# simonsobs/pixell

Measured on AMD Instinct MI355X. Metric: map2alm+alm2map round-trips/sec, higher is better.
Workload: dtype f64

## Files before the change

pixell_amd/csrc/leg_s0.hip:

```cpp
#include "legendre_dev.hpp"

namespace pxs {

#define S0_PHASE_A \
	while (k + 4 <= nk) { \
		bool act = false; \
		_Pragma("unroll") for (int s = 0; s < K; s++) act |= LEG_IS_LIVE(lam2[s], sc[s]); \
		if (__any(act)) break; \
		const double4_t q0 = LDC(coef, k), q1 = LDC(coef, k+1), q2 = LDC(coef, k+2), q3 = LDC(coef, k+3); \
		const double b0 = polar ? q0.c : q0.b, b1 = polar ? q1.c : q1.b, b2 = polar ? q2.c : q2.b, b3 = polar ? q3.c : q3.b; \
		_Pragma("unroll") for (int s = 0; s < K; s++) { \
			lam1[s] = fma(fma(q0.a, csq[s], b0), lam2[s], lam1[s]); \
			lam2[s] = fma(fma(q1.a, csq[s], b1), lam1[s], lam2[s]); \
			lam1[s] = fma(fma(q2.a, csq[s], b2), lam2[s], lam1[s]); \
			lam2[s] = fma(fma(q3.a, csq[s], b3), lam1[s], lam2[s]); \
			if (sc[s] < 0 && fabs(lam2[s]) > SC_BIG) { lam1[s] *= SC_SMALL; lam2[s] *= SC_SMALL; sc[s]++; } \
		} \
		k += 4; \
	}
#define S0_SEEDED_PHASE_A \
	if (a.seed_mode == 2) { \
		const double* sd = a.seed_d + ((long)m*a.nwave + wv)*(2*K*64); const int* si = a.seed_i + ((long)m*a.nwave + wv)*((K+1)*64); \
		k = PXS_UNIFORM_INT(si[K*64]); \
		_Pragma("unroll") for (int s = 0; s < K; s++) { lam1[s] = sd[s*64 + lane]; lam2[s] = sd[(K+s)*64 + lane]; sc[s] = si[s*64 + lane]; } \
	} else { \
		S0_PHASE_A \
		if (a.seed_mode == 1) { \
			double* sd = a.seed_d + ((long)m*a.nwave + wv)*(2*K*64); int* si = a.seed_i + ((long)m*a.nwave + wv)*((K+1)*64); \
			_Pragma("unroll") for (int s = 0; s < K; s++) { sd[s*64 + lane] = lam1[s]; sd[(K+s)*64 + lane] = lam2[s]; si[s*64 + lane] = sc[s]; } \
			if (lane == 0) si[K*64] = k; \
		} \
	}

#define S0_SYN_PAIR(c0, c1, a0, a1) S0_SYN_PAIR_C(c0.a, polar ? c0.c : c0.b, c1.a, polar ? c1.c : c1.b, a0, a1)
#define S0_SYN_PAIR_C(ca0, cb0, ca1, cb1, a0, a1) { \
	PXS_VCOPY(vb0, cb0); \
	PXS_VCOPY(vb1, cb1); \
	_Pragma("unroll") for (int s = 0; s < K; s++) { \
		p1r[s] = fma(lam2[s], a0.a, p1r[s]); p1i[s] = fma(lam2[s], a0.b, p1i[s]); \
		p2r[s] = fma(lam2[s], a0.c, p2r[s]); p2i[s] = fma(lam2[s], a0.d, p2i[s]); \
		lam1[s] = fma(fma(ca0, csq[s], vb0), lam2[s], lam1[s]); \
	} \
	_Pragma("unroll") for (int s = 0; s < K; s++) { \
		p1r[s] = fma(lam1[s], a1.a, p1r[s]); p1i[s] = fma(lam1[s], a1.b, p1i[s]); \
		p2r[s] = fma(lam1[s], a1.c, p2r[s]); p2i[s] = fma(lam1[s], a1.d, p2i[s]); \
		lam2[s] = fma(fma(ca1, csq[s], vb1), lam1[s], lam2[s]); \
	} }

template<int K> __global__ __launch_bounds__(64, (K == 4 ? 7 : 1)) void leg_syn_s0(const LegK a)
{
	const int lane = threadIdx.x; int wv, m, bb;
	if (!leg_block(a, wv, m, bb)) return;
	const long row0 = PXS_UNIFORM_LONG(a.row[m]);
	const int nk = (a.lmax - m)/2 + 1;
	const double4_t* __restrict__ coef = a.coef + row0;
	const double4_t* __restrict__ at = reinterpret_cast<const double4_t*>(a.almt + (long)bb*a.almt_bs) + row0;
	double x[K], csq[K], lam1[K], lam2[K], p1r[K], p1i[K], p2r[K], p2i[K];
	int sc[K], rn[K], rs[K];
	bool alive_any = false;
	const bool polar = leg_wave_polar(a, wv, K);
#pragma unroll
	for (int s = 0; s < K; s++) {
		const int p = leg_pair_u(a, wv, K, s, lane);
		const bool valid = leg_pair_valid(a, p);
		rn[s] = valid ? a.ring_n[p] : -1; rs[s] = valid ? a.ring_s[p] : -1;
		x[s] = valid ? a.cth[p] : 0.0;
		const double sth = valid ? a.sth[p] : 0.0;
		csq[s] = polar ? -sth*sth : x[s]*x[s];
		const bool alive = valid && ((double)m <= a.lmax*sth + a.ofs);
		lam1[s] = 0; lam2[s] = 0; sc[s] = 0;
		if (alive && a.seed_mode != 2) { double mt; int e; pow_scaled(sth, m, mt, e); to_scaled(mt, e, lam2[s], sc[s]); }
		p1r[s] = p1i[s] = p2r[s] = p2i[s] = 0;
		alive_any |= alive;
	}
	int k = 0;
	if (__any(alive_any)) {
		S0_SEEDED_PHASE_A
		k = PXS_UNIFORM_INT(k); coef = (const double4_t*)PXS_UNIFORM_LONG((long)coef);
		PXS_COUNT(0, (long)(nk - k)*K*6 + (a.seed_mode != 2 ? (long)k*K*2 : 0L));
		while (k + 1 < nk) {
			bool pend = false;
#pragma unroll
			for (int s = 0; s < K; s++) pend |= (sc[s] < 0);
			if (!__any(pend)) break;
			for (int it = 0; it < 2 && k + 1 < nk; it++, k += 2) {
				const double4_t c0 = LDC(coef, k), c1 = LDC(coef, k+1), a0 = LDC(at, k), a1 = LDC(at, k+1);
				S0_SYN_PAIR(c0, c1, a0, a1)
			}
#pragma unroll
			for (int s = 0; s < K; s++)
				if (sc[s] < 0 && fabs(lam2[s]) > SC_BIG) {
					lam1[s] *= SC_SMALL; lam2[s] *= SC_SMALL;
					if (++sc[s] == 0) p1r[s] = p1i[s] = p2r[s] = p2i[s] = 0;
				}
		}
#pragma unroll
		for (int s = 0; s < K; s++) if (sc[s] < 0) { p1r[s] = p1i[s] = p2r[s] = p2i[s] = 0; lam1[s] = lam2[s] = 0; }
		const double2* __restrict__ cf = (const double2*)PXS_UNIFORM_LONG((long)((polar ? a.coef2p : a.coef2) + row0));
		coef2x2_t f = LDC2(cf, k); double4_t a0 = LDC(at, k), a1 = LDC(at, k+1);
		while (k + 3 < nk) {
			PXS_ROWS_DRAIN();
			coef2x2_t n = LDC2(cf, k+2); double4_t m0 = LDC(at, k+2), m1 = LDC(at, k+3);
			PXS_ROWS_ISSUED();
			S0_SYN_PAIR_C(f.a0, f.b0, f.a1, f.b1, a0, a1)
			PXS_ROWS_DRAIN();
			f = LDC2(cf, k+4); a0 = LDC(at, k+4); a1 = LDC(at, k+5);
			PXS_ROWS_ISSUED();
			S0_SYN_PAIR_C(n.a0, n.b0, n.a1, n.b1, m0, m1)
			k += 4;
		}
		for (; k + 1 < nk; k += 2) {
			PXS_ROWS_DRAIN();
			const coef2x2_t n = LDC2(cf, k+2); const double4_t m0 = LDC(at, k+2), m1 = LDC(at, k+3);
			PXS_ROWS_ISSUED();
			S0_SYN_PAIR_C(f.a0, f.b0, f.a1, f.b1, a0, a1)
			f = n; a0 = m0; a1 = m1;
		}
		PXS_ROWS_DRAIN();
		if (k < nk) {
#pragma unroll
			for (int s = 0; s < K; s++) {
				p1r[s] = fma(lam2[s], a0.a, p1r[s]); p1i[s] = fma(lam2[s], a0.b, p1i[s]);
				p2r[s] = fma(lam2[s], a0.c, p2r[s]); p2i[s] = fma(lam2[s], a0.d, p2i[s]);
			}
		}
	}
	double2* __restrict__ out = a.leg + (long)bb*a.leg_bs + (long)m*a.ld;
#pragma unroll
	for (int s = 0; s < K; s++) {
		const int p = leg_pair_u(a, wv, K, s, lane);
		const bool valid = leg_pair_valid(a, p);
		const int rn_ = valid ? a.ring_n[p] : -1, rs_ = valid ? a.ring_s[p] : -1;
		const double x_ = valid ? a.cth[p] : 0.0;
		if (rn_ >= 0) out[rn_] = make_double2(p1r[s] + x_*p2r[s], p1i[s] + x_*p2i[s]);
		if (rs_ >= 0) out[rs_] = make_double2(p1r[s] - x_*p2r[s], p1i[s] - x_*p2i[s]);
	}
}

#define S0_ANA_PAIR(c0, c1) { \
	PXS_VCOPY(vb0, polar ? c0.c : c0.b); \
	PXS_VCOPY(vb1, polar ? c1.c : c1.b); \
	double t0 = 0, t1 = 0, t2 = 0, t3 = 0, u0 = 0, u1 = 0, u2 = 0, u3 = 0; \
	_Pragma("unroll") for (int s = 0; s < K; s++) { \
		t0 = fma(lam2[s], d1r[s], t0); t1 = fma(lam2[s], d1i[s], t1); t2 = fma(lam2[s], d2r[s], t2); t3 = fma(lam2[s], d2i[s], t3); \
		lam1[s] = fma(fma(c0.a, csq[s], vb0), lam2[s], lam1[s]); \
	} \
	_Pragma("unroll") for (int s = 0; s < K; s++) { \
		u0 = fma(lam1[s], d1r[s], u0); u1 = fma(lam1[s], d1i[s], u1); u2 = fma(lam1[s], d2r[s], u2); u3 = fma(lam1[s], d2i[s], u3); \
		lam2[s] = fma(fma(c1.a, csq[s], vb1), lam1[s], lam2[s]); \
	} \
	 \
	LEG_RED_PUT(kk, t0, t1, t2, t3) \
	LEG_RED_PUT(kk+1, u0, u1, u2, u3) \
	kk += 2; \
	if (kk == LEG_FSTEPS) { leg_flush(red, pout + 4*kbase, lane, LEG_FSTEPS, a.atomic); kk = 0; kbase = k+2; } }

#define S0_ANA_STEP_C(ca, cb, LA, LB, T0, T1, T2, T3) { \
	PXS_VCOPY(vb, cb); \
	_Pragma("unroll") for (int s = 0; s < K; s++) { \
		T0 = fma(LA[s], d1r[s], T0); T1 = fma(LA[s], d1i[s], T1); T2 = fma(LA[s], d2r[s], T2); T3 = fma(LA[s], d2i[s], T3); \
		LB[s] = fma(fma(ca, csq[s], vb), LA[s], LB[s]); \
	} }
#define S0_ANA_PAIR_D(ca0, cb0, ca1, cb1, kfirst, NEXT) { \
	double t0 = 0, t1 = 0, t2 = 0, t3 = 0, u0 = 0, u1 = 0, u2 = 0, u3 = 0; \
	S0_ANA_STEP_C(ca0, cb0, lam2, lam1, t0, t1, t2, t3) \
	_Pragma("unroll") for (int s = 0; s < K; s++) PXS_DONE(lam1[s]); \
	PXS_DONE(t0); PXS_DONE(t1); PXS_DONE(t2); PXS_DONE(t3); \
	PXS_ROWS_DRAIN(); \
	if (kk == LEG_FSTEPS) { leg_flush(red, pout + 4*kbase, lane, LEG_FSTEPS, a.atomic); kk = 0; kbase = (kfirst); } \
	NEXT; \
	PXS_ROWS_ISSUED(); \
	S0_ANA_STEP_C(ca1, cb1, lam1, lam2, u0, u1, u2, u3) \
	LEG_RED_PUT(kk, t0, t1, t2, t3) \
	LEG_RED_PUT(kk+1, u0, u1, u2, u3) \
	kk += 2; }

template<int K> __global__ __launch_bounds__(64) void leg_ana_s0(const LegK a)
{
	PXS_SHARED(double, red);
	const int lane = threadIdx.x; int wv, m, bb;
	if (!leg_block(a, wv, m, bb)) return;
	const long row0 = PXS_UNIFORM_LONG(a.row[m]);
	const int nk = (a.lmax - m)/2 + 1;
	const double4_t* __restrict__ coef = a.coef + row0;
	double* __restrict__ pout = a.part + (long)bb*a.mom_bs + ((long)wv*a.rows_chunk + (row0 - a.rowbase))*4;
	const double2* __restrict__ in = a.leg + (long)bb*a.leg_bs + (long)m*a.ld;
	double csq[K], lam1[K], lam2[K], d1r[K], d1i[K], d2r[K], d2i[K];
	int sc[K];
	bool alive_any = false;
	const bool polar = leg_wave_polar(a, wv, K);
	auto load_data = [&](int s) {
		const int p = leg_pair(a, wv, K, s, PXS_LATE_INT(lane));
		const bool valid = leg_pair_valid(a, p);
		const int rn = valid ? a.ring_n[p] : -1, rs = valid ? a.ring_s[p] : -1;
		const double x = valid ? a.cth[p] : 0.0;
		const double2 vn = rn >= 0 ? in[rn] : make_double2(0, 0);
		const double2 vs = rs >= 0 ? in[rs] : make_double2(0, 0);
		d1r[s] = vn.x + vs.x; d1i[s] = vn.y + vs.y;
		d2r[s] = (vn.x - vs.x)*x; d2i[s] = (vn.y - vs.y)*x;
	};
#pragma unroll
	for (int s = 0; s < K; s++) {
		const int p = leg_pair(a, wv, K, s, lane);
		const bool valid = leg_pair_valid(a, p);
		const double x = valid ? a.cth[p] : 0.0;
		const double sth = valid ? a.sth[p] : 0.0;
		csq[s] = polar ? -sth*sth : x*x;
		const bool alive = valid && ((double)m <= a.lmax*sth + a.ofs);
		lam1[s] = 0; lam2[s] = 0; sc[s] = 0;
		if (alive && a.seed_mode != 2) { double mt; int e; pow_scaled(sth, m, mt, e); to_scaled(mt, e, lam2[s], sc[s]); }
		d1r[s] = d1i[s] = d2r[s] = d2i[s] = 0;
		alive_any |= alive;
	}
	if (!__any(alive_any)) return;
	int k = 0;
	S0_SEEDED_PHASE_A
	k = PXS_UNIFORM_INT(k); coef = (const double4_t*)PXS_UNIFORM_LONG((long)coef);
	PXS_COUNT(1, (long)(nk - k)*K*6 + (a.seed_mode != 2 ? (long)k*K*2 : 0L));
	if (lane == 0 && !a.atomic) a.first[wv*a.nmc + (m - a.m0)] = k + 1;
#pragma unroll
	for (int s = 0; s < K; s++) if (sc[s] == 0) load_data(s);
	int kk = 0, kbase = k;
	while (k + 1 < nk) {
		bool pend = false;
#pragma unroll
		for (int s = 0; s < K; s++) pend |= (sc[s] < 0);
		if (!__any(pend)) break;
		for (int it = 0; it < 2 && k + 1 < nk; it++, k += 2) {
			const double4_t c0 = LDC(coef, k), c1 = LDC(coef, k+1);
			S0_ANA_PAIR(c0, c1)
		}
#pragma unroll
		for (int s = 0; s < K; s++)
			if (sc[s] < 0 && fabs(lam2[s]) > SC_BIG) {
				lam1[s] *= SC_SMALL; lam2[s] *= SC_SMALL;
				if (++sc[s] == 0) load_data(s);
			}
	}
	const double2* __restrict__ cf = (const double2*)PXS_UNIFORM_LONG((long)((polar ? a.coef2p : a.coef2) + row0));
	coef2x2_t n = LDC2(cf, k), f = LDC2(cf, k+1);
	PXS_ROWS_DRAIN();
	n.a1 = n.a0; n.b1 = n.b0;
	while (k + 3 < nk) {
		S0_ANA_PAIR_D(n.a1, n.b1, f.a0, f.b0, k, n = LDC2(cf, k+3))
		S0_ANA_PAIR_D(f.a1, f.b1, n.a0, n.b0, k+2, f = LDC2(cf, k+5))
		k += 4;
	}
	if (k + 1 < nk) {
		S0_ANA_PAIR_D(n.a1, n.b1, f.a0, f.b0, k, (void)0)
		k += 2;
	}
	PXS_ROWS_DRAIN();
	if (kk == LEG_FSTEPS) { leg_flush(red, pout + 4*kbase, lane, LEG_FSTEPS, a.atomic); kk = 0; kbase = k; }
	if (k < nk) {
		double t0 = 0, t1 = 0, t2 = 0, t3 = 0;
#pragma unroll
		for (int s = 0; s < K; s++) { t0 = fma(lam2[s], d1r[s], t0); t1 = fma(lam2[s], d1i[s], t1); t2 = fma(lam2[s], d2r[s], t2); t3 = fma(lam2[s], d2i[s], t3); }
		LEG_RED_PUT(kk, t0, t1, t2, t3)
		kk++;
	}
	if (kk > 0) leg_flush(red, pout + 4*kbase, lane, kk, a.atomic);
}


struct S0Chain {
	double csq, lam1, lam2; int sc;
	__device__ __forceinline__ double step(double ca, double cb) { const double p = lam2, nx = fma(mm_coef(ca, csq, cb), lam2, lam1); lam1 = p; lam2 = nx; return p; }
	__device__ __forceinline__ void rescale() { if (fabs(lam2) > SC_BIG) { lam1 *= SC_SMALL; lam2 *= SC_SMALL; sc++; } }
	__device__ __forceinline__ void park_sign(int, double*) const {}
};
struct S0Mm {
	typedef S0Chain Chain;
	static constexpr int SLOTS = 64;
	static constexpr bool SIGNED = false;
	static constexpr bool BREG_SYNC = true;
	static __device__ __forceinline__ int steps(const LegK& a, int m, int& par) { par = 0; return (a.lmax - m)/2 + 1; }
	static __device__ __forceinline__ bool init(const LegK& a, int p, int m, int, bool polar, S0Chain& C) {
		const bool valid = p < a.npairs;
		const double x = valid ? a.cth[p] : 0.0, sth = valid ? a.sth[p] : 0.0;
		C.csq = polar ? -sth*sth : x*x;
		const bool alive = valid && ((double)m <= a.lmax*sth + a.ofs);
		C.lam1 = 0; C.lam2 = 0; C.sc = 0;
		if (alive) { double mt; int e; pow_scaled(sth, m, mt, e); to_scaled(mt, e, C.lam2, C.sc); }
		return alive;
	}
	static __device__ __forceinline__ const double* table(const LegK& a, bool polar, long row0) { return reinterpret_cast<const double*>(polar ? a.coef2p : a.coef2) + 2*row0; }
	static __device__ __forceinline__ int phase_a(const LegK& a, S0Chain& C, long row0, bool polar, int nk) {
		const double4_t* __restrict__ coef = a.coef + row0;
		int k = 0;
		while (k + 4 <= nk) {
			if (__any(LEG_IS_LIVE(C.lam2, C.sc))) break;
			const double4_t q0 = LDC(coef, k), q1 = LDC(coef, k+1), q2 = LDC(coef, k+2), q3 = LDC(coef, k+3);
			const double b0 = polar ? q0.c : q0.b, b1 = polar ? q1.c : q1.b, b2 = polar ? q2.c : q2.b, b3 = polar ? q3.c : q3.b;
			C.lam1 = fma(fma(q0.a, C.csq, b0), C.lam2, C.lam1);
			C.lam2 = fma(fma(q1.a, C.csq, b1), C.lam1, C.lam2);
			C.lam1 = fma(fma(q2.a, C.csq, b2), C.lam2, C.lam1);
			C.lam2 = fma(fma(q3.a, C.csq, b3), C.lam1, C.lam2);
			if (C.sc < 0) C.rescale();
			k += 4;
		}
		return k;
	}
	struct Data { double2 vn[4], vs[4]; };
	static __device__ __forceinline__ void load(const LegK& a, int m, int map0, int rn, int rs, Data& d) {
#pragma unroll
		for (int mm = 0; mm < 4; mm++) {
			const int map = map0 + mm;
			const double2* __restrict__ in = a.leg + (long)map*a.leg_bs + (long)m*a.ld;
			const bool okm = map < a.nmaps;
			d.vn[mm] = (okm && rn >= 0) ? in[rn] : make_double2(0, 0); d.vs[mm] = (okm && rs >= 0) ? in[rs] : make_double2(0, 0);
		}
	}
	static __device__ __forceinline__ void park(const Data& d, double x, int, double* __restrict__ ent) {
#pragma unroll
		for (int mm = 0; mm < 4; mm++) {
			ent[4*mm + 0] = d.vn[mm].x + d.vs[mm].x; ent[4*mm + 1] = d.vn[mm].y + d.vs[mm].y;
			ent[4*mm + 2] = (d.vn[mm].x - d.vs[mm].x)*x; ent[4*mm + 3] = (d.vn[mm].y - d.vs[mm].y)*x;
		}
	}
	template<int NG> static __device__ __forceinline__ void store(const LegK& a, int m, int bb, int pbase, int lane, mm_acc (&acc)[NG][4]) {
		const int c = lane & 3;
#pragma unroll
		for (int g = 0; g < NG; g++) {
			const int map = (bb*NG + g)*4 + ((lane & 15) >> 2);
			double* __restrict__ out = reinterpret_cast<double*>(a.leg + (long)(map < a.nmaps ? map : 0)*a.leg_bs + (long)m*a.ld) + (c & 1);
#pragma unroll
			for (int rb = 0; rb < 4; rb++)
#pragma unroll
				for (int r = 0; r < 4; r++) {
					const int p = pbase + 16*rb + 4*r + (lane >> 4);
					const bool valid = p < a.npairs && map < a.nmaps;
					const double v = acc[g][rb][r], o = MMS_XOR2(v);
					const double x = valid ? a.cth[p] : 0.0;
					const double val = c < 2 ? fma(x, o, v) : fma(-x, v, o);
					const int ring = valid ? (c < 2 ? a.ring_n[p] : a.ring_s[p]) : -1;
					if (ring >= 0) out[2*ring] = val;
				}
		}
	}
};
template<int NG, int W> __global__ __launch_bounds__(64*W, 4) void leg_ana_s0_mm(const LegK a) { leg_ana_mm<S0Mm, NG, W>(a); }



template<int NG> __global__ __launch_bounds__(64, 4) void leg_syn_s0_mm(const LegK a) { leg_syn_mm<S0Mm, NG>(a); }

void launch_leg_s0(bool analysis, int ng, int K, dim3 grid, hipStream_t st, const LegK& a) {
	static const bool once = leg_mm_lds_optin({leg_ana_s0_mm<2, MM_WAVES>, leg_ana_s0_mm<1, MM_WAVES>}); (void)once;
	const LegKernel k = analysis ? (ng == 2 ? leg_ana_s0_mm<2, MM_WAVES> : ng ? leg_ana_s0_mm<1, MM_WAVES> : K == 8 ? leg_ana_s0<8> : K == 4 ? leg_ana_s0<4> : K == 2 ? leg_ana_s0<2> : nullptr)
	                             : (ng == 2 ? leg_syn_s0_mm<2> : ng ? leg_syn_s0_mm<1> : K == 4 ? leg_syn_s0<4> : K == 2 ? leg_syn_s0<2> : nullptr);
	PXS_REQUIRE(k != nullptr, "internal: no spin-0 Legendre kernel compiled for this number of ring pairs per lane");
	leg_launch(k, analysis, ng, grid, st, a);
}

}
```

pixell_amd/csrc/leg_spin.hip:

```cpp
#include "legendre_dev.hpp"

namespace pxs {

template<int K> struct SpinState {
	double x[K], gp1[K], gp2[K], gm1[K], gm2[K];
	int scp[K], scm[K];
};

template<int K> __device__ __forceinline__ bool spin_init(const LegK& a, int wv, int lane, int m, SpinState<K>& S, int* rn, int* rs, bool polar) {
	const int s_ = a.spin;
	bool alive_any = false;
#pragma unroll
	for (int s = 0; s < K; s++) {
		const int p = leg_pair(a, wv, K, s, lane);
		const bool valid = leg_pair_valid(a, p);
		rn[s] = valid ? a.ring_n[p] : -1; rs[s] = valid ? a.ring_s[p] : -1;
		const double cth = valid ? a.cth[p] : 0.0;
		const double sth = valid ? a.sth[p] : 0.0;
		const double shh = valid ? a.sh2[p] : 0.0;
		S.x[s] = polar ? -2.0*shh*shh : cth;
		const double t1 = a.lmax*sth + a.ofs;
		const double b = -2.0*s_*fabs(cth);
		const double c = (double)s_*s_ - t1*t1;
		const double discr = b*b - 4*c;
		const double mlim = discr <= 0 ? a.lmax : fmin((double)a.lmax, 0.5*(-b + sqrt(discr)));
		const bool alive = valid && ((double)m <= mlim + 0.5);
		S.gp1[s] = S.gm1[s] = 0; S.gp2[s] = S.gm2[s] = 0; S.scp[s] = S.scm[s] = 0;
		if (alive && a.seed_mode != 2) {
			const double sh = shh, ch = a.ch2[p];
			double m1, m2; int e1, e2;
			if (m >= s_) {
				pow_scaled(sh, m + s_, m1, e1); pow_scaled(ch, m - s_, m2, e2);
				double mt = m1*m2; int e = e1 + e2 + m; frexp_norm(mt, e); to_scaled(mt, e, S.gp2[s], S.scp[s]);
				pow_scaled(sh, m - s_, m1, e1); pow_scaled(ch, m + s_, m2, e2);
				mt = m1*m2; e = e1 + e2 + m; frexp_norm(mt, e); to_scaled(mt, e, S.gm2[s], S.scm[s]);
			} else {
				pow_scaled(sh, s_ + m, m1, e1); pow_scaled(ch, s_ - m, m2, e2);
				double mt = m1*m2; int e = e1 + e2; frexp_norm(mt, e); to_scaled(mt, e, S.gp2[s], S.scp[s]);
				pow_scaled(sh, s_ - m, m1, e1); pow_scaled(ch, s_ + m, m2, e2);
				mt = m1*m2; e = e1 + e2; frexp_norm(mt, e); to_scaled(mt, e, S.gm2[s], S.scm[s]);
				if ((s_ - m) & 1) S.gm2[s] = -S.gm2[s];
			}
		}
		alive_any |= alive;
	}
	return alive_any;
}

#define SPIN_PHASE_A \
	while (j + 4 <= nl) { \
		bool act = false; \
		_Pragma("unroll") for (int s = 0; s < K; s++) act |= LEG_IS_LIVE(S.gp2[s], S.scp[s]) || LEG_IS_LIVE(S.gm2[s], S.scm[s]); \
		if (__any(act)) break; \
		const double4_t q0 = LDC(coef, j), q1 = LDC(coef, j+1), q2 = LDC(coef, j+2), q3 = LDC(coef, j+3); \
		_Pragma("unroll") for (int s = 0; s < K; s++) { \
			double ax; \
			ax = q0.a*S.x[s]; S.gp1[s] = fma(ax + (polar ? q0.c : q0.b), S.gp2[s], -S.gp1[s]); S.gm1[s] = fma(ax + (polar ? q0.d : -q0.b), S.gm2[s], -S.gm1[s]); \
			ax = q1.a*S.x[s]; S.gp2[s] = fma(ax + (polar ? q1.c : q1.b), S.gp1[s], -S.gp2[s]); S.gm2[s] = fma(ax + (polar ? q1.d : -q1.b), S.gm1[s], -S.gm2[s]); \
			ax = q2.a*S.x[s]; S.gp1[s] = fma(ax + (polar ? q2.c : q2.b), S.gp2[s], -S.gp1[s]); S.gm1[s] = fma(ax + (polar ? q2.d : -q2.b), S.gm2[s], -S.gm1[s]); \
			ax = q3.a*S.x[s]; S.gp2[s] = fma(ax + (polar ? q3.c : q3.b), S.gp1[s], -S.gp2[s]); S.gm2[s] = fma(ax + (polar ? q3.d : -q3.b), S.gm1[s], -S.gm2[s]); \
			if (S.scp[s] < 0 && fabs(S.gp2[s]) > SC_BIG) { S.gp1[s] *= SC_SMALL; S.gp2[s] *= SC_SMALL; S.scp[s]++; } \
			if (S.scm[s] < 0 && fabs(S.gm2[s]) > SC_BIG) { S.gm1[s] *= SC_SMALL; S.gm2[s] *= SC_SMALL; S.scm[s]++; } \
		} \
		j += 4; \
	}

#define SPIN_SEEDED_PHASE_A \
	if (a.seed_mode == 2) { \
		const double* sd = a.seed_d + ((long)m*a.nwave + wv)*(4*K*64); const int* si = a.seed_i + ((long)m*a.nwave + wv)*((2*K+1)*64); \
		j = PXS_UNIFORM_INT(si[2*K*64]); \
		_Pragma("unroll") for (int s = 0; s < K; s++) { \
			S.gp1[s] = sd[s*64 + lane]; S.gp2[s] = sd[(K+s)*64 + lane]; S.gm1[s] = sd[(2*K+s)*64 + lane]; S.gm2[s] = sd[(3*K+s)*64 + lane]; \
			S.scp[s] = si[s*64 + lane]; S.scm[s] = si[(K+s)*64 + lane]; } \
	} else { \
		SPIN_PHASE_A \
		if (a.seed_mode == 1) { \
			double* sd = a.seed_d + ((long)m*a.nwave + wv)*(4*K*64); int* si = a.seed_i + ((long)m*a.nwave + wv)*((2*K+1)*64); \
			_Pragma("unroll") for (int s = 0; s < K; s++) { \
				sd[s*64 + lane] = S.gp1[s]; sd[(K+s)*64 + lane] = S.gp2[s]; sd[(2*K+s)*64 + lane] = S.gm1[s]; sd[(3*K+s)*64 + lane] = S.gm2[s]; \
				si[s*64 + lane] = S.scp[s]; si[(K+s)*64 + lane] = S.scm[s]; } \
			if (lane == 0) si[2*K*64] = j; \
		} \
	}

struct spin_rows_t { double4_t r0, r1; };
__device__ __forceinline__ spin_rows_t spin_rows(const double4_t* coef, long i) { spin_rows_t r; r.r0 = LDC(coef, i); r.r1 = LDC(coef, i+1); return r; }
#define SPIN_ROW0(r) r.r0.a, polar ? r.r0.c : r.r0.b, polar ? r.r0.d : -r.r0.b
#define SPIN_ROW1(r) r.r1.a, polar ? r.r1.c : r.r1.b, polar ? r.r1.d : -r.r1.b

#define SPIN_SYN_PAIR(f0, f1, a0, a1) SPIN_SYN_PAIR_C(f0.a, polar ? f0.c : f0.b, polar ? f0.d : -f0.b, f1.a, polar ? f1.c : f1.b, polar ? f1.d : -f1.b, a0, a1)
#define SPIN_SYN_PAIR_C(ca0, c10, c20, ca1, c11, c21, a0, a1) { \
	{ \
		const double ca = ca0, c1 = c10, c2 = c20; \
		PXS_VCOPY(v1, c1); PXS_VCOPY(v2, c2); \
		_Pragma("unroll") for (int s = 0; s < K; s++) { \
			const double gp = S.gp2[s], gm = S.gm2[s]; \
			pnr[s] = fma(gp, a0.a, pnr[s]); pni[s] = fma(gp, a0.b, pni[s]); \
			mnr[s] = fma(gm, a0.c, mnr[s]); mni[s] = fma(gm, a0.d, mni[s]); \
			qsr[s] = fma(gm, a0.a, qsr[s]); qsi[s] = fma(gm, a0.b, qsi[s]); \
			nsr[s] = fma(gp, a0.c, nsr[s]); nsi[s] = fma(gp, a0.d, nsi[s]); \
			S.gp1[s] = fma(fma(ca, S.x[s], v1), gp, -S.gp1[s]); S.gm1[s] = fma(fma(ca, S.x[s], v2), gm, -S.gm1[s]); \
		} \
	} \
	{ \
		const double ca = ca1, c1 = c11, c2 = c21; \
		PXS_VCOPY(v1, c1); PXS_VCOPY(v2, c2); \
		_Pragma("unroll") for (int s = 0; s < K; s++) { \
			const double gp = S.gp1[s], gm = S.gm1[s]; \
			pnr[s] = fma(gp, a1.a, pnr[s]); pni[s] = fma(gp, a1.b, pni[s]); \
			mnr[s] = fma(gm, a1.c, mnr[s]); mni[s] = fma(gm, a1.d, mni[s]); \
			qsr[s] = fma(-gm, a1.a, qsr[s]); qsi[s] = fma(-gm, a1.b, qsi[s]); \
			nsr[s] = fma(-gp, a1.c, nsr[s]); nsi[s] = fma(-gp, a1.d, nsi[s]); \
			S.gp2[s] = fma(fma(ca, S.x[s], v1), gp, -S.gp2[s]); S.gm2[s] = fma(fma(ca, S.x[s], v2), gm, -S.gm2[s]); \
		} \
	} }

#define SPIN_SYN_PAIR_R(s0, s1, a0, a1) SPIN_SYN_PAIR_C(s0, s1, a0, a1)
#define SPIN_SYN_PHASE_C { \
	spin_rows_t f = spin_rows(coef, j); a0 = LDC(at, j); a1 = LDC(at, j+1); \
	while (j + 3 < nl) { \
		PXS_ROWS_DRAIN(); \
		spin_rows_t n = spin_rows(coef, j+2); double4_t m0 = LDC(at, j+2), m1 = LDC(at, j+3); \
		PXS_ROWS_ISSUED(); \
		SPIN_SYN_PAIR_R(SPIN_ROW0(f), SPIN_ROW1(f), a0, a1) \
		PXS_ROWS_DRAIN(); \
		f = spin_rows(coef, j+4); a0 = LDC(at, j+4); a1 = LDC(at, j+5); \
		PXS_ROWS_ISSUED(); \
		SPIN_SYN_PAIR_R(SPIN_ROW0(n), SPIN_ROW1(n), m0, m1) \
		j += 4; \
	} \
	for (; j + 1 < nl; j += 2) { \
		PXS_ROWS_DRAIN(); \
		const spin_rows_t n = spin_rows(coef, j+2); const double4_t m0 = LDC(at, j+2), m1 = LDC(at, j+3); \
		PXS_ROWS_ISSUED(); \
		SPIN_SYN_PAIR_R(SPIN_ROW0(f), SPIN_ROW1(f), a0, a1) \
		f = n; a0 = m0; a1 = m1; \
	} \
	PXS_ROWS_DRAIN(); }

template<int K> __global__ __launch_bounds__(64) void leg_syn_spin(const LegK a)
{
	const int lane = threadIdx.x; int wv, m, bb;
	if (!leg_block(a, wv, m, bb)) return;
	const int l0 = max(m, a.spin);
	const int nl = a.lmax - l0 + 1;
	double2* __restrict__ outq = a.leg + (long)bb*a.leg_bs + (long)m*a.ld;
	double2* __restrict__ outu = a.leg + (long)bb*a.leg_bs + ((long)a.nm + m)*a.ld;
	SpinState<K> S; int rn[K], rs[K];
	double pnr[K], pni[K], mnr[K], mni[K], qsr[K], qsi[K], nsr[K], nsi[K];
#pragma unroll
	for (int s = 0; s < K; s++) pnr[s] = pni[s] = mnr[s] = mni[s] = qsr[s] = qsi[s] = nsr[s] = nsi[s] = 0;
	const bool polar = leg_wave_polar(a, wv, K);
	const bool alive_any = spin_init<K>(a, wv, lane, m, S, rn, rs, polar);
	double sg0 = 1.0;
	if (nl > 0 && __any(alive_any)) {
		const long row0 = PXS_UNIFORM_LONG(a.row[m]);
		const double4_t* __restrict__ coef = a.coef + row0;
		const double4_t* __restrict__ at = reinterpret_cast<const double4_t*>(a.almt + (long)bb*a.almt_bs) + row0;
		int j = 0;
		SPIN_SEEDED_PHASE_A
		j = PXS_UNIFORM_INT(j); coef = (const double4_t*)PXS_UNIFORM_LONG((long)coef);
		PXS_COUNT(0, (long)(nl - j)*K*12 + (a.seed_mode != 2 ? (long)j*K*4 : 0L));
		sg0 = ((l0 + j + m) & 1) ? -1.0 : 1.0;
		while (j + 1 < nl) {
			bool pend = false;
#pragma unroll
			for (int s = 0; s < K; s++) pend |= (S.scp[s] < 0) || (S.scm[s] < 0);
			if (!__any(pend)) break;
			for (int it = 0; it < 2 && j + 1 < nl; it++, j += 2) {
				const double4_t f0 = LDC(coef, j), f1 = LDC(coef, j+1), a0 = LDC(at, j), a1 = LDC(at, j+1);
				SPIN_SYN_PAIR(f0, f1, a0, a1)
			}
#pragma unroll
			for (int s = 0; s < K; s++) {
				const bool was = (S.scp[s] < 0) || (S.scm[s] < 0);
				if (S.scp[s] < 0 && fabs(S.gp2[s]) > SC_BIG) { S.gp1[s] *= SC_SMALL; S.gp2[s] *= SC_SMALL; S.scp[s]++; }
				if (S.scm[s] < 0 && fabs(S.gm2[s]) > SC_BIG) { S.gm1[s] *= SC_SMALL; S.gm2[s] *= SC_SMALL; S.scm[s]++; }
				if (was && S.scp[s] == 0 && S.scm[s] == 0) pnr[s] = pni[s] = mnr[s] = mni[s] = qsr[s] = qsi[s] = nsr[s] = nsi[s] = 0;
			}
		}
#pragma unroll
		for (int s = 0; s < K; s++)
			if (S.scp[s] < 0 || S.scm[s] < 0) {
				pnr[s] = pni[s] = mnr[s] = mni[s] = qsr[s] = qsi[s] = nsr[s] = nsi[s] = 0;
				S.gp1[s] = S.gp2[s] = S.gm1[s] = S.gm2[s] = 0;
			}
		double4_t a0, a1;
		SPIN_SYN_PHASE_C
		if (j < nl) {
#pragma unroll
			for (int s = 0; s < K; s++) {
				const double gp = S.gp2[s], gm = S.gm2[s];
				pnr[s] = fma(gp, a0.a, pnr[s]); pni[s] = fma(gp, a0.b, pni[s]);
				mnr[s] = fma(gm, a0.c, mnr[s]); mni[s] = fma(gm, a0.d, mni[s]);
				qsr[s] = fma(gm, a0.a, qsr[s]); qsi[s] = fma(gm, a0.b, qsi[s]);
				nsr[s] = fma(gp, a0.c, nsr[s]); nsi[s] = fma(gp, a0.d, nsi[s]);
			}
		}
	}
#pragma unroll
	for (int s = 0; s < K; s++) {
		const int p = leg_pair(a, wv, K, s, lane);
		const bool valid = leg_pair_valid(a, p);
		const int rn_ = valid ? a.ring_n[p] : -1, rs_ = valid ? a.ring_s[p] : -1;
		if (rn_ >= 0) {
			outq[rn_] = make_double2(0.5*(pnr[s] + mnr[s]), 0.5*(pni[s] + mni[s]));
			outu[rn_] = make_double2(0.5*(pni[s] - mni[s]), -0.5*(pnr[s] - mnr[s]));
		}
		if (rs_ >= 0) {
			const double psr = sg0*qsr[s], psi = sg0*qsi[s], msr = sg0*nsr[s], msi = sg0*nsi[s];
			outq[rs_] = make_double2(0.5*(psr + msr), 0.5*(psi + msi));
			outu[rs_] = make_double2(0.5*(psi - msi), -0.5*(psr - msr));
		}
	}
}

#define SPIN_ANA_PAIR(f0, f1) { \
	double t0 = 0, t1 = 0, t2 = 0, t3 = 0, u0 = 0, u1 = 0, u2 = 0, u3 = 0; \
	{ \
		const double ca = f0.a, c1 = polar ? f0.c : f0.b, c2 = polar ? f0.d : -f0.b; \
		PXS_VCOPY(v1, c1); PXS_VCOPY(v2, c2); \
		_Pragma("unroll") for (int s = 0; s < K; s++) { \
			const double gp = S.gp2[s], gm = S.gm2[s]; \
			t0 = fma(gp, tpnr[s], t0); t0 = fma(gm, tpsr[s], t0); \
			t1 = fma(gp, tpni[s], t1); t1 = fma(gm, tpsi[s], t1); \
			t2 = fma(gm, tmnr[s], t2); t2 = fma(gp, tmsr[s], t2); \
			t3 = fma(gm, tmni[s], t3); t3 = fma(gp, tmsi[s], t3); \
			S.gp1[s] = fma(fma(ca, S.x[s], v1), gp, -S.gp1[s]); S.gm1[s] = fma(fma(ca, S.x[s], v2), gm, -S.gm1[s]); \
		} \
	} \
	{ \
		const double ca = f1.a, c1 = polar ? f1.c : f1.b, c2 = polar ? f1.d : -f1.b; \
		PXS_VCOPY(v1, c1); PXS_VCOPY(v2, c2); \
		_Pragma("unroll") for (int s = 0; s < K; s++) { \
			const double gp = S.gp1[s], gm = S.gm1[s]; \
			u0 = fma(gp, tpnr[s], u0); u0 = fma(-gm, tpsr[s], u0); \
			u1 = fma(gp, tpni[s], u1); u1 = fma(-gm, tpsi[s], u1); \
			u2 = fma(gm, tmnr[s], u2); u2 = fma(-gp, tmsr[s], u2); \
			u3 = fma(gm, tmni[s], u3); u3 = fma(-gp, tmsi[s], u3); \
			S.gp2[s] = fma(fma(ca, S.x[s], v1), gp, -S.gp2[s]); S.gm2[s] = fma(fma(ca, S.x[s], v2), gm, -S.gm2[s]); \
		} \
	} \
	 \
	LEG_RED_PUT(kk, t0, t1, t2, t3) \
	LEG_RED_PUT(kk+1, u0, u1, u2, u3) \
	kk += 2; \
	if (kk == LEG_FSTEPS) { leg_flush(red, pout + 4*jbase, lane, LEG_FSTEPS, a.atomic); kk = 0; jbase = j+2; } }

#define SPIN_ANA_STEP0_C(ca, c1, c2) { \
	PXS_VCOPY(v1, c1); PXS_VCOPY(v2, c2); \
	_Pragma("unroll") for (int s = 0; s < K; s++) { \
		const double gp = S.gp2[s], gm = S.gm2[s]; \
		t0 = fma(gp, tpnr[s], t0); t0 = fma(gm, tpsr[s], t0); \
		t1 = fma(gp, tpni[s], t1); t1 = fma(gm, tpsi[s], t1); \
		t2 = fma(gm, tmnr[s], t2); t2 = fma(gp, tmsr[s], t2); \
		t3 = fma(gm, tmni[s], t3); t3 = fma(gp, tmsi[s], t3); \
		S.gp1[s] = fma(fma(ca, S.x[s], v1), gp, -S.gp1[s]); S.gm1[s] = fma(fma(ca, S.x[s], v2), gm, -S.gm1[s]); \
	} }
#define SPIN_ANA_STEP1_C(ca, c1, c2) { \
	PXS_VCOPY(v1, c1); PXS_VCOPY(v2, c2); \
	_Pragma("unroll") for (int s = 0; s < K; s++) { \
		const double gp = S.gp1[s], gm = S.gm1[s]; \
		u0 = fma(gp, tpnr[s], u0); u0 = fma(-gm, tpsr[s], u0); \
		u1 = fma(gp, tpni[s], u1); u1 = fma(-gm, tpsi[s], u1); \
		u2 = fma(gm, tmnr[s], u2); u2 = fma(-gp, tmsr[s], u2); \
		u3 = fma(gm, tmni[s], u3); u3 = fma(-gp, tmsi[s], u3); \
		S.gp2[s] = fma(fma(ca, S.x[s], v1), gp, -S.gp2[s]); S.gm2[s] = fma(fma(ca, S.x[s], v2), gm, -S.gm2[s]); \
	} }
#define SPIN_ANA_PAIR_D(ca0, c10, c20, ca1, c11, c21, jfirst, NEXT) { \
	double t0 = 0, t1 = 0, t2 = 0, t3 = 0, u0 = 0, u1 = 0, u2 = 0, u3 = 0; \
	SPIN_ANA_STEP0_C(ca0, c10, c20) \
	_Pragma("unroll") for (int s = 0; s < K; s++) { PXS_DONE(S.gp1[s]); PXS_DONE(S.gm1[s]); } \
	PXS_DONE(t0); PXS_DONE(t1); PXS_DONE(t2); PXS_DONE(t3); \
	PXS_ROWS_DRAIN(); \
	if (kk == LEG_FSTEPS) { leg_flush(red, pout + 4*jbase, lane, LEG_FSTEPS, a.atomic); kk = 0; jbase = (jfirst); } \
	NEXT; \
	PXS_ROWS_ISSUED(); \
	SPIN_ANA_STEP1_C(ca1, c11, c21) \
	LEG_RED_PUT(kk, t0, t1, t2, t3) \
	LEG_RED_PUT(kk+1, u0, u1, u2, u3) \
	kk += 2; }
#define SPIN_ANA_PHASE_C { \
	spin_rows_t n = spin_rows(coef, j), f = spin_rows(coef, j+1); \
	PXS_ROWS_DRAIN(); \
	n.r1 = n.r0; \
	while (j + 3 < nl) {       \
		SPIN_ANA_PAIR_R(SPIN_ROW1(n), SPIN_ROW0(f), j, n = spin_rows(coef, j+3)) \
		SPIN_ANA_PAIR_R(SPIN_ROW1(f), SPIN_ROW0(n), j+2, f = spin_rows(coef, j+5)) \
		j += 4; \
	} \
	if (j + 1 < nl) { \
		SPIN_ANA_PAIR_R(SPIN_ROW1(n), SPIN_ROW0(f), j, (void)0) \
		j += 2; \
	} }
#define SPIN_ANA_PAIR_R(s0, s1, jfirst, NEXT) SPIN_ANA_PAIR_D(s0, s1, jfirst, NEXT)

template<int K> __global__ __launch_bounds__(64, (K == 2 ? 5 : 1)) void leg_ana_spin(const LegK a)
{
	PXS_SHARED(double, red);
	const int lane = threadIdx.x; int wv, m, bb;
	if (!leg_block(a, wv, m, bb)) return;
	const int l0 = max(m, a.spin);
	const int nl = a.lmax - l0 + 1;
	if (nl <= 0) return;
	const long row0 = PXS_UNIFORM_LONG(a.row[m]);
	const double4_t* __restrict__ coef = a.coef + row0;
	double* __restrict__ pout = a.part + (long)bb*a.mom_bs + ((long)wv*a.rows_chunk + (row0 - a.rowbase))*4;
	const double2* __restrict__ inq = a.leg + (long)bb*a.leg_bs + (long)m*a.ld;
	const double2* __restrict__ inu = a.leg + (long)bb*a.leg_bs + ((long)a.nm + m)*a.ld;
	SpinState<K> S; int rn[K], rs[K];
	const bool polar = leg_wave_polar(a, wv, K);
	const bool alive_any = spin_init<K>(a, wv, lane, m, S, rn, rs, polar);
	if (!__any(alive_any)) return;
	const double sgn0 = ((l0 + m) & 1) ? -1.0 : 1.0;
	double tpnr[K], tpni[K], tmnr[K], tmni[K], tpsr[K], tpsi[K], tmsr[K], tmsi[K];
	auto load_data = [&](int s) {
		const int p = leg_pair(a, wv, K, s, PXS_LATE_INT(lane));
		const bool valid = leg_pair_valid(a, p);
		const int rn_ = valid ? a.ring_n[p] : -1, rs_ = valid ? a.ring_s[p] : -1;
		double2 q = rn_ >= 0 ? inq[rn_] : make_double2(0, 0), u = rn_ >= 0 ? inu[rn_] : make_double2(0, 0);
		tpnr[s] = q.x - u.y; tpni[s] = q.y + u.x; tmnr[s] = q.x + u.y; tmni[s] = q.y - u.x;
		q = rs_ >= 0 ? inq[rs_] : make_double2(0, 0); u = rs_ >= 0 ? inu[rs_] : make_double2(0, 0);
		tpsr[s] = sgn0*(q.x - u.y); tpsi[s] = sgn0*(q.y + u.x); tmsr[s] = sgn0*(q.x + u.y); tmsi[s] = sgn0*(q.y - u.x);
	};
#pragma unroll
	for (int s = 0; s < K; s++) tpnr[s] = tpni[s] = tmnr[s] = tmni[s] = tpsr[s] = tpsi[s] = tmsr[s] = tmsi[s] = 0;
	int j = 0;
	SPIN_SEEDED_PHASE_A
	j = PXS_UNIFORM_INT(j); coef = (const double4_t*)PXS_UNIFORM_LONG((long)coef);
	PXS_COUNT(1, (long)(nl - j)*K*12 + (a.seed_mode != 2 ? (long)j*K*4 : 0L));
	if (lane == 0 && !a.atomic) a.first[wv*a.nmc + (m - a.m0)] = j + 1;
#pragma unroll
	for (int s = 0; s < K; s++) if (S.scp[s] == 0 && S.scm[s] == 0) load_data(s);
	int kk = 0, jbase = j;
	while (j + 1 < nl) {
		bool pend = false;
#pragma unroll
		for (int s = 0; s < K; s++) pend |= (S.scp[s] < 0) || (S.scm[s] < 0);
		if (!__any(pend)) break;
		for (int it = 0; it < 2 && j + 1 < nl; it++, j += 2) {
			const double4_t f0 = LDC(coef, j), f1 = LDC(coef, j+1);
			SPIN_ANA_PAIR(f0, f1)
		}
#pragma unroll
		for (int s = 0; s < K; s++) {
			const bool was = (S.scp[s] < 0) || (S.scm[s] < 0);
			if (S.scp[s] < 0 && fabs(S.gp2[s]) > SC_BIG) { S.gp1[s] *= SC_SMALL; S.gp2[s] *= SC_SMALL; S.scp[s]++; }
			if (S.scm[s] < 0 && fabs(S.gm2[s]) > SC_BIG) { S.gm1[s] *= SC_SMALL; S.gm2[s] *= SC_SMALL; S.scm[s]++; }
			if (was && S.scp[s] == 0 && S.scm[s] == 0) load_data(s);
		}
	}
	SPIN_ANA_PHASE_C
	PXS_ROWS_DRAIN();
	if (kk == LEG_FSTEPS) { leg_flush(red, pout + 4*jbase, lane, LEG_FSTEPS, a.atomic); kk = 0; jbase = j; }
	if (j < nl) {
		double t0 = 0, t1 = 0, t2 = 0, t3 = 0;
#pragma unroll
		for (int s = 0; s < K; s++) {
			const double gp = S.gp2[s], gm = S.gm2[s];
			t0 = fma(gp, tpnr[s], t0); t0 = fma(gm, tpsr[s], t0);
			t1 = fma(gp, tpni[s], t1); t1 = fma(gm, tpsi[s], t1);
			t2 = fma(gm, tmnr[s], t2); t2 = fma(gp, tmsr[s], t2);
			t3 = fma(gm, tmni[s], t3); t3 = fma(gp, tmsi[s], t3);
		}
		LEG_RED_PUT(kk, t0, t1, t2, t3)
		kk++;
	}
	if (kk > 0) leg_flush(red, pout + 4*jbase, lane, kk, a.atomic);
}


struct SpinChain {
	double x, g1, g2, sgl, pa; int sc, half, par;
	__device__ __forceinline__ double coef(double ca, double cb) const { return fma(ca, x, fma(sgl, cb, pa*ca)); }
	__device__ __forceinline__ double step(double ca, double cb) { const double p = g2, nx = fma(coef(ca, cb), g2, -g1); g1 = p; g2 = nx; return p; }
	__device__ __forceinline__ void rescale() { if (fabs(g2) > SC_BIG) { g1 *= SC_SMALL; g2 *= SC_SMALL; sc++; } }
	__device__ __forceinline__ void park_sign(int kq, double* p) const {
		const double se = (half && ((par + kq) & 1)) ? -1.0 : 1.0, so = half ? -se : 1.0;
		p[0] *= se; p[1] *= so; p[2] *= se; p[3] *= so;
	}
};
struct SpinMm {
	typedef SpinChain Chain;
	static constexpr int SLOTS = 32;
	static constexpr bool SIGNED = true;
	static constexpr bool BREG_SYNC = false;
	static __device__ __forceinline__ int steps(const LegK& a, int m, int& par) { const int l0 = max(m, a.spin); par = l0 + m; return a.lmax - l0 + 1; }
	static __device__ __forceinline__ bool init(const LegK& a, int p, int m, int half, bool polar, SpinChain& C) {
		const int s_ = a.spin;
		const bool valid = p < a.npairs;
		const double cth = valid ? a.cth[p] : 0.0, sth = valid ? a.sth[p] : 0.0, shh = valid ? a.sh2[p] : 0.0;
		C.x = polar ? -2.0*shh*shh : cth; C.sgl = half ? -1.0 : 1.0; C.pa = polar ? 1.0 : 0.0; C.half = half; C.par = max(m, s_) + m;
		const double t1 = a.lmax*sth + a.ofs, b = -2.0*s_*fabs(cth), c = (double)s_*s_ - t1*t1, discr = b*b - 4*c;
		const double mlim = discr <= 0 ? a.lmax : fmin((double)a.lmax, 0.5*(-b + sqrt(discr)));
		const bool alive = valid && ((double)m <= mlim + 0.5);
		C.g1 = 0; C.g2 = 0; C.sc = 0;
		if (alive) {
			const double sh = shh, ch = a.ch2[p];
			double m1, m2; int e1, e2;
			const int es = m >= s_ ? (half ? m - s_ : m + s_) : (half ? s_ - m : s_ + m), ec = m >= s_ ? (half ? m + s_ : m - s_) : (half ? s_ + m : s_ - m);
			pow_scaled(sh, es, m1, e1); pow_scaled(ch, ec, m2, e2);
			double mt = m1*m2; int e = e1 + e2 + (m >= s_ ? m : 0); frexp_norm(mt, e); to_scaled(mt, e, C.g2, C.sc);
			if (m < s_ && half && ((s_ - m) & 1)) C.g2 = -C.g2;
		}
		return alive;
	}
	static __device__ __forceinline__ const double* table(const LegK& a, bool, long row0) { return reinterpret_cast<const double*>(a.coef2) + 2*row0; }
	static __device__ __forceinline__ int phase_a(const LegK& a, SpinChain& C, long row0, bool polar, int n) {
		const double* __restrict__ tab = table(a, polar, row0);
		int k = 0;
		while (k + 4 <= n) {
			if (__any(LEG_IS_LIVE(C.g2, C.sc))) break;
			double cq[8];
#pragma unroll
			for (int i = 0; i < 8; i++) cq[i] = LDCD(tab, 2L*k + i);
#pragma unroll
			for (int i = 0; i < 4; i++) C.step(cq[2*i], cq[2*i + 1]);
			if (C.sc < 0) C.rescale();
			k += 4;
		}
		return k;
	}
	struct Data { double2 qn[4], un[4], qs[4], us[4]; };
	static __device__ __forceinline__ void load(const LegK& a, int m, int map0, int rn, int rs, Data& d) {
#pragma unroll
		for (int mm = 0; mm < 4; mm++) {
			const int map = map0 + mm;
			const double2* __restrict__ inq = a.leg + (long)map*a.leg_bs + (long)m*a.ld;
			const double2* __restrict__ inu = a.leg + (long)map*a.leg_bs + ((long)a.nm + m)*a.ld;
			const bool okm = map < a.nmaps;
			d.qn[mm] = (okm && rn >= 0) ? inq[rn] : make_double2(0, 0); d.un[mm] = (okm && rn >= 0) ? inu[rn] : make_double2(0, 0);
			d.qs[mm] = (okm && rs >= 0) ? inq[rs] : make_double2(0, 0); d.us[mm] = (okm && rs >= 0) ? inu[rs] : make_double2(0, 0);
		}
	}
	static __device__ __forceinline__ void park(const Data& d, double, int half, double* __restrict__ ent) {
#pragma unroll
		for (int mm = 0; mm < 4; mm++) {
			const double tpn_r = d.qn[mm].x - d.un[mm].y, tpn_i = d.qn[mm].y + d.un[mm].x, tmn_r = d.qn[mm].x + d.un[mm].y, tmn_i = d.qn[mm].y - d.un[mm].x;
			const double tps_r = d.qs[mm].x - d.us[mm].y, tps_i = d.qs[mm].y + d.us[mm].x, tms_r = d.qs[mm].x + d.us[mm].y, tms_i = d.qs[mm].y - d.us[mm].x;
			ent[4*mm + 0] = half ? tps_r : tpn_r; ent[4*mm + 1] = half ? tps_i : tpn_i;
			ent[4*mm + 2] = half ? tmn_r : tms_r; ent[4*mm + 3] = half ? tmn_i : tms_i;
		}
	}
	template<int NG> static __device__ __forceinline__ void store(const LegK& a, int m, int bb, int pbase, int lane, mm_acc (&acc)[NG][4]) {
		const int c = lane & 3;
#pragma unroll
		for (int g = 0; g < NG; g++) {
			const int map = (bb*NG + g)*4 + ((lane & 15) >> 2);
			double* __restrict__ outq = reinterpret_cast<double*>(a.leg + (long)(map < a.nmaps ? map : 0)*a.leg_bs + (long)m*a.ld);
			double* __restrict__ outu = reinterpret_cast<double*>(a.leg + (long)(map < a.nmaps ? map : 0)*a.leg_bs + ((long)a.nm + m)*a.ld);
#pragma unroll
			for (int rb = 0; rb < 2; rb++)
#pragma unroll
				for (int r = 0; r < 4; r++) {
					const int p = pbase + 16*rb + 4*r + (lane >> 4);
					const bool valid = p < a.npairs && map < a.nmaps;
					const double own = acc[g][rb][r], oth = MMS_XOR2(acc[g][rb + 2][r]);
					const double P = c < 2 ? own : oth, M = c < 2 ? oth : own;
					const double sum = 0.5*(P + M), dif = 0.5*(P - M);
					const int ring = valid ? (c < 2 ? a.ring_n[p] : a.ring_s[p]) : -1;
					if (ring >= 0) {
						if (c & 1) { outq[2*ring + 1] = sum; outu[2*ring] = dif; }
						else       { outq[2*ring] = sum; outu[2*ring + 1] = -dif; }
					}
				}
		}
	}
};
template<int NG, int W> __global__ __launch_bounds__(64*W, 4) void leg_ana_spin_mm(const LegK a) { leg_ana_mm<SpinMm, NG, W>(a); }

template<int NG> __global__ __launch_bounds__(64, 4) void leg_syn_spin_mm(const LegK a) { leg_syn_mm<SpinMm, NG>(a); }

void launch_leg_spin(bool analysis, int ng, int K, dim3 grid, hipStream_t st, const LegK& a) {
	static const bool once = leg_mm_lds_optin({leg_ana_spin_mm<2, MM_WAVES>, leg_ana_spin_mm<1, MM_WAVES>}); (void)once;
	const LegKernel k = analysis ? (ng == 2 ? leg_ana_spin_mm<2, MM_WAVES> : ng ? leg_ana_spin_mm<1, MM_WAVES> : K == 6 ? leg_ana_spin<6> : K == 4 ? leg_ana_spin<4> : K == 3 ? leg_ana_spin<3> : K == 2 ? leg_ana_spin<2> : nullptr)
	                             : (ng == 2 ? leg_syn_spin_mm<2> : ng ? leg_syn_spin_mm<1> : K == 3 ? leg_syn_spin<3> : K == 2 ? leg_syn_spin<2> : nullptr);
	PXS_REQUIRE(k != nullptr, "internal: no spin-s Legendre kernel compiled for this number of ring pairs per lane");
	leg_launch(k, analysis, ng, grid, st, a);
}

}
```

pixell_amd/csrc/legendre_dev.hpp:

```cpp
#pragma once
#include "legendre.hpp"
#include <cmath>
#include <algorithm>
#include <initializer_list>

namespace pxs {

static constexpr double SC_BIG   = 0x1p+400;
static constexpr double SC_SMALL = 0x1p-800;
static constexpr int    SC_STEP  = 800;
static constexpr double LEG_LIVE = 0x1p-140;
#define LEG_IS_LIVE(v, sc) ((sc) == 0 && fabs(v) >= LEG_LIVE)

struct double4_t { double a, b, c, d; };
#ifdef PXS_HOST_SIM
#define LDC(p, i) ((p)[i])
#else
typedef double pxs_d4 __attribute__((ext_vector_type(4)));
__device__ __forceinline__ double4_t ldc_row(const double4_t* p, long i) {
	const __attribute__((address_space(4))) pxs_d4* c = (const __attribute__((address_space(4))) pxs_d4*)(unsigned long long)p;
	const pxs_d4 v = c[i]; double4_t r; r.a = v.x; r.b = v.y; r.c = v.z; r.d = v.w; return r;
}
#define LDC(p, i) ldc_row((p), (i))
#endif
#ifdef PXS_HOST_SIM
#define LDCD(p, i) ((p)[i])
#else
__device__ __forceinline__ double ldc_double(const double* p, long i) {
	const __attribute__((address_space(4))) double* c = (const __attribute__((address_space(4))) double*)(unsigned long long)p;
	return c[i];
}
#define LDCD(p, i) ldc_double((p), (i))
#endif

struct coef2x2_t { double a0, b0, a1, b1; };
#ifdef PXS_HOST_SIM
#define LDC2(p, i) (coef2x2_t{(p)[i].x, (p)[i].y, (p)[(i)+1].x, (p)[(i)+1].y})
#define PXS_ROWS_DRAIN()
#define PXS_ROWS_ISSUED()
#else
typedef double pxs_d4a16 __attribute__((ext_vector_type(4), aligned(16)));
__device__ __forceinline__ coef2x2_t ldc_row2(const double2* p, long i) {
	const __attribute__((address_space(4))) pxs_d4a16* c = (const __attribute__((address_space(4))) pxs_d4a16*)(unsigned long long)(p + i);
	const pxs_d4a16 v = *c; coef2x2_t r; r.a0 = v.x; r.b0 = v.y; r.a1 = v.z; r.b1 = v.w; return r;
}
#define LDC2(p, i) ldc_row2((p), (i))
#define PXS_ROWS_DRAIN() do { __builtin_amdgcn_s_waitcnt(0xc07f); __builtin_amdgcn_sched_barrier(0); } while (0)
#define PXS_ROWS_ISSUED() __builtin_amdgcn_sched_barrier(0)
#endif
#ifdef PXS_HOST_SIM
#define PXS_DONE(x)
#else
#define PXS_DONE(x) asm volatile("" : "+v"(x))
#endif

struct LegK {
	int lmax, mmax, spin, nm, npairs, nring, nwave;
	long ld;
	long nrows;
	const long* row; const double4_t* coef; const double* alpha;
	const int* ring_n; const int* ring_s; const double* cth; const double* sth; const double* sh2; const double* ch2;
	double* almt; double* part; double* mom;
	double2* leg;
	double ofs;
	int m0; long rowbase, rows_chunk;
	int nmc, xcd;
	int* first;
	int atomic;
	int seed_mode; double* seed_d; int* seed_i;
	double* count;
	int nb; long leg_bs, almt_bs, mom_bs;
	int nmaps;
	const double2* coef2; const double2* coef2p;
};
#define PXS_NCOUNT 1024
#ifdef PXS_HOST_SIM
#define PXS_COUNT(dir, expr) if (a.count != nullptr && lane == 0) atomicAdd(a.count + 2*(blockIdx.x & (PXS_NCOUNT - 1)) + (dir), (double)(expr))
#else
#define PXS_COUNT(dir, expr) if (a.count != nullptr && lane == 0) unsafeAtomicAdd(a.count + 2*(blockIdx.x & (PXS_NCOUNT - 1)) + (dir), (double)(expr))
#endif

__host__ __device__ constexpr unsigned leg_blocks_per_m(unsigned nwave, unsigned nb) { return (nwave*nb) | 1u; }
static_assert(leg_blocks_per_m(20, 1) == 21 && leg_blocks_per_m(27, 1) == 27 && leg_blocks_per_m(4, 8) == 33 && leg_blocks_per_m(3, 2) == 7, "blocks per m: odd, at most one more than chunks x maps");
__device__ __forceinline__ bool leg_block(const LegK& a, int& wv, int& m, int& bb) {
	if (!a.xcd) { wv = blockIdx.x; m = blockIdx.y + a.m0; bb = blockIdx.z; return true; }
	const unsigned b = blockIdx.x, x = b & 7u, j = b >> 3;
	const unsigned per_m = leg_blocks_per_m((unsigned)a.nwave, (unsigned)a.nb);
	const unsigned ml = j / per_m, r = j - ml*per_m;
	bb = (int)(r / (unsigned)a.nwave);
	wv = (int)(r - (unsigned)bb*a.nwave);
	const unsigned mi = ml*8u + x;
	m = (int)mi + a.m0;
	return mi < (unsigned)a.nmc && bb < a.nb;
}
static inline dim3 leg_grid(const LegK& a) { return a.xcd ? dim3((unsigned)(8*((a.nmc+7)/8)*leg_blocks_per_m(a.nwave, a.nb))) : dim3(a.nwave, a.nmc, a.nb); }

__device__ __forceinline__ void frexp_norm(double& m, int& e) { int d; m = frexp(m, &d); e += d; }

__device__ __forceinline__ void pow_scaled(double x, int n, double& mant, int& e) {
	double rm = 0.5; int re = 1;
	int be = 0; double bm = frexp(x, &be);
	while (n) {
		if (n & 1) { rm *= bm; re += be; frexp_norm(rm, re); }
		bm *= bm; be *= 2; frexp_norm(bm, be);
		n >>= 1;
	}
	mant = rm; e = re;
}
__device__ __forceinline__ void to_scaled(double mant, int e, double& v, int& scale) {
	if (mant == 0.0) { v = 0.0; scale = 0; return; }
	int s = (e >= 0) ? (e + SC_STEP/2)/SC_STEP : -((-e + SC_STEP/2)/SC_STEP);
	if (s > 0) s = 0;
	v = ldexp(mant, e - SC_STEP*s); scale = s;
}

#ifndef PXS_POLAR_COS2
#define PXS_POLAR_COS2 0.1
#endif
__device__ __forceinline__ bool mm_wave_polar(const LegK& a, int end) {
	const double c = a.cth[min(end, a.npairs) - 1];
	return c*c > PXS_POLAR_COS2;
}
__host__ __device__ constexpr int leg_pair_of(int npairs, int nwave, int K, int wv, int s, int lane) { return (wv*K + s)*64 + lane - (nwave*K*64 - npairs); }
__host__ __device__ constexpr int leg_wave_last_pair(int npairs, int K, int wv) { return leg_pair_of(npairs, (npairs + 64*K - 1)/(64*K), K, wv, K - 1, 63); }
static_assert(leg_wave_last_pair(1451, 3, 0) == 106 && leg_wave_last_pair(1451, 4, 0) == 170 && leg_wave_last_pair(1451, 8, 0) == 426, "pair map: first wave");
static_assert(leg_wave_last_pair(1451, 3, 7) == 1450 && leg_wave_last_pair(1451, 4, 5) == 1450 && leg_wave_last_pair(1451, 8, 2) == 1450, "pair map: last wave");
static_assert(leg_pair_of(1451, 8, 3, 0, 0, 0) == -85 && leg_pair_of(1451, 8, 3, 0, 1, 21) == 0 && leg_pair_of(512, 2, 4, 0, 0, 0) == 0 && leg_wave_last_pair(30, 4, 0) == 29, "pair map: padding");
__device__ __forceinline__ int leg_pair(const LegK& a, int wv, int K, int s, int lane) { return leg_pair_of(a.npairs, a.nwave, K, wv, s, lane); }
__device__ __forceinline__ bool leg_pair_valid(const LegK& a, int p) { return (unsigned)p < (unsigned)a.npairs; }
__device__ __forceinline__ bool leg_wave_polar(const LegK& a, int wv, int K) { return mm_wave_polar(a, leg_wave_last_pair(a.npairs, K, wv) + 1); }

#ifdef PXS_HOST_SIM
#define PXS_VCOPY(dst, src) double dst = (src)
#else
#define PXS_VCOPY(dst, src) double dst; asm("v_mov_b64 %0, %1" : "=v"(dst) : "s"(src))
#endif

#ifdef PXS_HOST_SIM
#define PXS_FRESH_INT(x) (x)
#else
__device__ __forceinline__ int pxs_fresh_int(int x) { asm("" : "+v"(x)); return x; }
#define PXS_FRESH_INT(x) pxs_fresh_int(x)
#endif
#ifdef PXS_HOST_SIM
#define PXS_LATE_INT(x) (x)
#else
__device__ __forceinline__ int pxs_late_int(int x) { asm volatile("" : "+v"(x)); return x; }
#define PXS_LATE_INT(x) pxs_late_int(x)
#endif


#ifdef PXS_HOST_SIM
#define PXS_UNIFORM_INT(x) (x)
#define PXS_UNIFORM_LONG(x) (x)
#else
#define PXS_UNIFORM_INT(x) __builtin_amdgcn_readfirstlane(x)
#define PXS_UNIFORM_LONG(x) ((long)(((unsigned long)(unsigned)__builtin_amdgcn_readfirstlane((int)((unsigned long)(x) >> 32)) << 32) | (unsigned long)(unsigned)__builtin_amdgcn_readfirstlane((int)(unsigned long)(x))))
#endif
__device__ __forceinline__ int leg_pair_u(const LegK& a, int wv, int K, int s, int lane) { return PXS_UNIFORM_INT(leg_pair(a, wv, K, s, 0)) + lane; }


#ifdef PXS_HOST_SIM
#define PXS_WAVE_LDS_SYNC() pxsim::wave_sync()
#else
#define PXS_WAVE_LDS_SYNC() asm volatile("s_waitcnt lgkmcnt(0)" ::: "memory")
#endif
#define LEG_FSTEPS 16
#ifdef PXS_HOST_SIM
#define LEG_RED_STRIDE 66
#define LEG_RED_DOUBLES (4*LEG_FSTEPS*LEG_RED_STRIDE)
__device__ __forceinline__ double leg_flush_sum(const double* red, int lane) {
	const double* r = red + lane*LEG_RED_STRIDE;
	double s0 = 0, s1 = 0, s2 = 0, s3 = 0;
	for (int i = 0; i < 64; i += 4) { s0 += r[i]; s1 += r[i+1]; s2 += r[i+2]; s3 += r[i+3]; }
	return (s0 + s1) + (s2 + s3);
}
__device__ __forceinline__ int leg_flush_col(int lane) { return lane; }
#define LEG_RED_PUT(kk, t0, t1, t2, t3) \
	red[((kk)*4+0)*LEG_RED_STRIDE + lane] = t0; red[((kk)*4+1)*LEG_RED_STRIDE + lane] = t1; \
	red[((kk)*4+2)*LEG_RED_STRIDE + lane] = t2; red[((kk)*4+3)*LEG_RED_STRIDE + lane] = t3;
#else
#define LEG_RED_STRIDE 18
#define LEG_RED_DOUBLES (4*LEG_FSTEPS*LEG_RED_STRIDE)
__device__ __forceinline__ void leg_swap32(double& a, double& b) {
	const unsigned alo = __double2loint(a), ahi = __double2hiint(a), blo = __double2loint(b), bhi = __double2hiint(b);
	const auto r0 = __builtin_amdgcn_permlane32_swap(alo, blo, false, false);
	const auto r1 = __builtin_amdgcn_permlane32_swap(ahi, bhi, false, false);
	a = __hiloint2double(r1[0], r0[0]); b = __hiloint2double(r1[1], r0[1]);
}
__device__ __forceinline__ void leg_swap16(double& a, double& b) {
	const unsigned alo = __double2loint(a), ahi = __double2hiint(a), blo = __double2loint(b), bhi = __double2hiint(b);
	const auto r0 = __builtin_amdgcn_permlane16_swap(alo, blo, false, false);
	const auto r1 = __builtin_amdgcn_permlane16_swap(ahi, bhi, false, false);
	a = __hiloint2double(r1[0], r0[0]); b = __hiloint2double(r1[1], r0[1]);
}
__device__ __forceinline__ double leg_flush_sum(const double* red, int lane) {
	const double2* r = reinterpret_cast<const double2*>(red + lane*LEG_RED_STRIDE);
	double sum = 0;
#pragma unroll 1
	for (int h = 0; h < 8; h += 4) {
		const double2 a = r[h], b = r[h+1], c = r[h+2], d = r[h+3];
		sum += ((a.x + a.y) + (b.x + b.y)) + ((c.x + c.y) + (d.x + d.y));
	}
	return sum;
}
__device__ __forceinline__ int leg_flush_col(int lane) { const int r = lane & 3; return (lane & ~3) | ((r == 1) ? 2 : (r == 2) ? 1 : r); }
#define LEG_RED_PUT(kk, t0, t1, t2, t3) { \
	double a_ = t0, b_ = t1, c_ = t2, d_ = t3; \
	leg_swap32(a_, b_); leg_swap32(c_, d_); \
	double u_ = a_ + b_, v_ = c_ + d_; \
	leg_swap16(u_, v_); \
	red[((kk)*4 + (lane >> 4))*LEG_RED_STRIDE + (lane & 15)] = u_ + v_; }
#endif
__device__ __forceinline__ void leg_flush(double* red, double* __restrict__ dst, int lane, int nkk, int atomic) {
	PXS_WAVE_LDS_SYNC();
	if (lane < 4*nkk) {
		const double sum = leg_flush_sum(red, lane);
		double* q = dst + leg_flush_col(lane);
#ifdef PXS_HOST_SIM
		if (atomic) atomicAdd(q, sum); else *q = sum;
#else
		if (atomic) unsafeAtomicAdd(q, sum); else *q = sum;
#endif
	}
	PXS_WAVE_LDS_SYNC();
}


#define MM_PSTRIDE 65
#define MM_WAVES 8
#define MM_ESTRIDE 17
#ifdef PXS_HOST_SIM
struct mm_acc { double v[4]; double& operator[](int i) { return v[i]; } };
static inline mm_acc mm_mfma(double av, double bv, mm_acc c) {
	pxsim::BlockCtx* cx = pxsim::t_ctx; const int w = pxsim::wave_id(), l = pxsim::lane_id();
	uint64_t* s = cx->wslot->data() + (size_t)w*128;
	memcpy(&s[l], &av, 8); memcpy(&s[64 + l], &bv, 8); cx->wbar[w]->wait();
	for (int r = 0; r < 4; r++) {
		const int i = 4*r + (l >> 4), j = l & 15;
		double sum = c.v[r];
		for (int kk = 0; kk < 4; kk++) { double x, y; memcpy(&x, &s[i + 16*kk], 8); memcpy(&y, &s[64 + j + 16*kk], 8); sum = fma(x, y, sum); }
		c.v[r] = sum;
	}
	cx->wbar[w]->wait();
	return c;
}
static inline void mm_lds_add(double* p, double v) { atomicAdd(p, v); }
#define MM_WAVE_SYNC() pxsim::t_ctx->wbar[pxsim::wave_id()]->wait()
#else
typedef double mm_acc __attribute__((ext_vector_type(4)));
__device__ __forceinline__ mm_acc mm_mfma(double av, double bv, mm_acc c) { return __builtin_amdgcn_mfma_f64_16x16x4f64(av, bv, c, 0, 0, 0); }
__device__ __forceinline__ void mm_lds_add(double* p, double v) { (void)__hip_atomic_fetch_add(p, v, __ATOMIC_RELAXED, __HIP_MEMORY_SCOPE_WORKGROUP); }
#define MM_WAVE_SYNC() asm volatile("s_waitcnt lgkmcnt(0)" ::: "memory")
#endif
__device__ __forceinline__ double mm_coef(double ca, double x2, double cb) { PXS_VCOPY(vb_, cb); return fma(ca, x2, vb_); }
__device__ __forceinline__ void mm_load_cf(double (&cf)[32], const double* __restrict__ tab, int k0) {
#pragma unroll
	for (int i = 0; i < 32; i++) cf[i] = LDCD(tab, 2L*k0 + i);
}
template<int STRIDE, class Chain>
__device__ __forceinline__ void mm_park_tile(Chain& C, const double (&cf)[32], int k0, int kw, int n, bool& pend, double* __restrict__ ptile, int lane) {
#pragma unroll
	for (int q4 = 0; q4 < 4; q4++) {
		const int kq = k0 + 4*q4;
		double p[4] = {0, 0, 0, 0};
		if (kq >= kw && kq < n) {
#pragma unroll
			for (int i = 0; i < 4; i++) p[i] = C.step(cf[8*q4 + 2*i], cf[8*q4 + 2*i + 1]);
			if (pend) {
				if (C.sc < 0) { p[0] = p[1] = p[2] = p[3] = 0.0; C.rescale(); }
				pend = __any(C.sc < 0);
			}
			C.park_sign(kq, p);
			if (kq + 1 >= n) p[1] = 0.0;
			if (kq + 2 >= n) p[2] = 0.0;
			if (kq + 3 >= n) p[3] = 0.0;
		}
#pragma unroll
		for (int i = 0; i < 4; i++) ptile[(4*q4 + i)*STRIDE + lane] = p[i];
	}
}
template<int NG, bool SIGNED> struct MmSynB {
	const double* src[NG]; bool ok[NG]; int kk4, cc, par;
	__device__ __forceinline__ void init(const LegK& a, int bb, long row0, int lane, int par_) {
		const int jcol = lane & 15; kk4 = lane >> 4; cc = jcol & 3; par = par_;
#pragma unroll
		for (int g = 0; g < NG; g++) {
			const int map = (bb*NG + g)*4 + (jcol >> 2);
			ok[g] = map < a.nmaps;
			src[g] = a.almt + (long)(ok[g] ? map : 0)*a.almt_bs + 4*row0 + cc + 16*kk4;
		}
	}
	__device__ __forceinline__ void load(int k0, int n, double (*b)[4]) const {
#pragma unroll
		for (int g = 0; g < NG; g++)
#pragma unroll
			for (int q = 0; q < 4; q++) {
				const int row = k0 + q + 4*kk4;
				const double v = (ok[g] && row < n) ? src[g][4L*(k0 + q)] : 0.0;
				b[g][q] = (SIGNED && cc >= 2 && ((par + row) & 1)) ? -v : v;
			}
	}
};
template<int NG, int W, bool SIGNED>
__device__ __forceinline__ void mm_flush(const LegK& a, double* __restrict__ red, int tf, int w, int lane, int bb, int n, long row0, int par) {
	double* __restrict__ redf = red + (tf & 1)*NG*4*64;
	for (int cidx = w; cidx < 4*NG; cidx += W) {
		const int g = cidx >> 2, r = cidx & 3;
		double* rp = redf + cidx*64 + lane;
		double v = *rp; *rp = 0.0;
		const int krow = 16*tf + 4*r + (lane >> 4), map = (bb*NG + g)*4 + ((lane & 15) >> 2), c = lane & 3;
		if (krow < n && map < a.nmaps) {
			if (SIGNED && c >= 2 && ((par + krow) & 1)) v = -v;
			double* dst = a.mom + (long)map*a.mom_bs + 4*(row0 + krow) + c;
#ifdef PXS_HOST_SIM
			atomicAdd(dst, v);
#else
			unsafeAtomicAdd(dst, v);
#endif
		}
	}
}
__host__ __device__ constexpr int mm_lds_doubles(int NG, int W) { return W*16*MM_PSTRIDE + 2*NG*4*64 > 64*W*MM_ESTRIDE ? W*16*MM_PSTRIDE + 2*NG*4*64 : 64*W*MM_ESTRIDE; }
static inline size_t mm_ana_lds(int NG, int W) { return sizeof(double)*(size_t)mm_lds_doubles(NG, W) + 16; }

#define MMS_PSTRIDE 68
static inline size_t mm_syn_lds() { return sizeof(double)*16*MMS_PSTRIDE; }
#ifdef PXS_HOST_SIM
#define MMS_XOR2(v) __shfl_xor((v), 2)
#else
__device__ __forceinline__ double mms_xor2(double v) {
	const int lo = __builtin_amdgcn_mov_dpp(__double2loint(v), 0x4e, 0xf, 0xf, true), hi = __builtin_amdgcn_mov_dpp(__double2hiint(v), 0x4e, 0xf, 0xf, true);
	return __hiloint2double(hi, lo);
}
#define MMS_XOR2(v) mms_xor2(v)
#endif

template<class Sys, int NG, int W> __device__ __forceinline__ void leg_ana_mm(const LegK& a)
{
	PXS_SHARED(double, sh);
	double* __restrict__ ptile = sh;
	double* __restrict__ red = sh + W*16*MM_PSTRIDE;
	int* __restrict__ s_kmin = reinterpret_cast<int*>(sh + mm_lds_doubles(NG, W));
	const int tid = threadIdx.x, lane = tid & 63, w = PXS_UNIFORM_INT(tid >> 6), half = lane/Sys::SLOTS;
	int wv, m, bb;
	if (!leg_block(a, wv, m, bb)) return;
	int par;
	const int n = Sys::steps(a, m, par);
	if (n <= 0) return;
	const long row0 = PXS_UNIFORM_LONG(a.row[m]);
	const int pbase = wv*Sys::SLOTS*W;
	const bool polar = mm_wave_polar(a, pbase + Sys::SLOTS*(w + 1));
	const int pmine_ = pbase + Sys::SLOTS*w + (lane & (Sys::SLOTS - 1));
	typename Sys::Chain C;
	const bool alive = Sys::init(a, pmine_, m, half, polar, C);
	if (tid == 0) *s_kmin = n;
	__syncthreads();
	const bool wave_alive = __any(alive);
	const int kw = PXS_UNIFORM_INT(wave_alive ? Sys::phase_a(a, C, row0, polar, n) : n + 16);
	if (lane == 0) atomicMin(s_kmin, kw);
	__syncthreads();
	const int kmin = PXS_UNIFORM_INT(*s_kmin);
	if (kmin >= n) return;
	double breg[NG][16];
	{
		const bool ok = pmine_ < a.npairs;
		const int rn = ok ? a.ring_n[pmine_] : -1, rs = ok ? a.ring_s[pmine_] : -1;
		const double x = ok ? a.cth[pmine_] : 0.0;
		double* __restrict__ ent = sh + tid*MM_ESTRIDE;
		const double* __restrict__ rd = sh + (64*w + 16*(lane >> 4))*MM_ESTRIDE + (lane & 15);
#pragma unroll
		for (int g = 0; g < NG; g++) {
			typename Sys::Data d;
			Sys::load(a, m, (bb*NG + g)*4, rn, rs, d);
			if (g > 0) __syncthreads();
			Sys::park(d, x, half, ent);
			__syncthreads();
#pragma unroll
			for (int q = 0; q < 16; q++) breg[g][q] = rd[q*MM_ESTRIDE];
			if (Sys::BREG_SYNC) MM_WAVE_SYNC();
		}
		__syncthreads();
		for (int i = tid; i < 2*NG*4*64; i += 64*W) red[i] = 0.0;
		__syncthreads();
	}
	const double* __restrict__ tab = Sys::table(a, polar, row0);
	bool pend = __any(C.sc < 0);
	double* __restrict__ pmine = ptile + w*16*MM_PSTRIDE;
	const double* __restrict__ pread = pmine + (lane & 15)*MM_PSTRIDE + 16*(lane >> 4);
	double cf[32]; int cf_tile = -1;
	long ntile = 0;
	auto flush = [&](int tf) { mm_flush<NG, W, Sys::SIGNED>(a, red, tf, w, lane, bb, n, row0, par); };
	int tlast = -1;
	for (int t = kmin >> 4; 16*t < n; t++) {
		const int k0 = 16*t;
		double* __restrict__ redt = red + (t & 1)*NG*4*64;
		if (k0 + 16 > kw) {
			ntile++;
			if (cf_tile != t) mm_load_cf(cf, tab, k0);
			mm_park_tile<MM_PSTRIDE>(C, cf, k0, kw, n, pend, pmine, lane);
			MM_WAVE_SYNC();
			double av[4];
#pragma unroll
			for (int q = 0; q < 4; q++) av[q] = pread[q];
			MM_WAVE_SYNC();
			if (k0 + 16 < n) { mm_load_cf(cf, tab, k0 + 16); cf_tile = t + 1; }
			mm_acc acc[NG];
#pragma unroll
			for (int g = 0; g < NG; g++) { acc[g][0] = 0; acc[g][1] = 0; acc[g][2] = 0; acc[g][3] = 0; }
#pragma unroll
			for (int q = 0; q < 16; q++) {
				const double aq = q < 4 ? av[q] : pread[q];
#pragma unroll
				for (int g = 0; g < NG; g++) acc[g] = mm_mfma(aq, breg[g][q], acc[g]);
			}
			if (tlast >= 0) { flush(tlast); tlast = -1; }
#pragma unroll
			for (int g = 0; g < NG; g++)
#pragma unroll
				for (int r = 0; r < 4; r++) mm_lds_add(redt + (g*4 + r)*64 + lane, acc[g][r]);
		}
		if (tlast >= 0) flush(tlast);
		tlast = t;
		__syncthreads();
	}
	if (tlast >= 0) flush(tlast);
	PXS_COUNT(1, ntile*(NG*256L + 32L) + (wave_alive ? (long)kw*2 : 0L));
}

template<class Sys, int NG> __device__ __forceinline__ void leg_syn_mm(const LegK& a)
{
	PXS_SHARED(double, pmine);
	const int lane = threadIdx.x, half = lane/Sys::SLOTS;
	int wv, m, bb;
	if (!leg_block(a, wv, m, bb)) return;
	int par;
	const int n = Sys::steps(a, m, par);
	const long row0 = PXS_UNIFORM_LONG(a.row[m]);
	const int pbase = wv*Sys::SLOTS;
	const bool polar = mm_wave_polar(a, pbase + Sys::SLOTS);
	typename Sys::Chain C;
	const bool alive = Sys::init(a, pbase + (lane & (Sys::SLOTS - 1)), m, half, polar, C);
	mm_acc acc[NG][4];
#pragma unroll
	for (int g = 0; g < NG; g++)
#pragma unroll
		for (int rb = 0; rb < 4; rb++) { acc[g][rb][0] = 0; acc[g][rb][1] = 0; acc[g][rb][2] = 0; acc[g][rb][3] = 0; }
	long ntile = 0;
	const bool wave_alive = n > 0 && __any(alive);
	const int kw = PXS_UNIFORM_INT(wave_alive ? Sys::phase_a(a, C, row0, polar, n) : max(n, 0) + 16);
	{
		const double* __restrict__ tab = Sys::table(a, polar, row0);
		MmSynB<NG, Sys::SIGNED> B; B.init(a, bb, row0, lane, par);
		bool pend = __any(C.sc < 0);
		const double* __restrict__ pread = pmine + 4*(lane >> 4)*MMS_PSTRIDE + (lane & 15);
		double cf[32];
		double bcur[NG][4], bnxt[NG][4];
		B.load(16*(kw >> 4), n, bcur);
		if (kw < n) mm_load_cf(cf, tab, 16*(kw >> 4));
		for (int t = kw >> 4; 16*t < n; t++) {
			const int k0 = 16*t;
			ntile++;
			mm_park_tile<MMS_PSTRIDE>(C, cf, k0, kw, n, pend, pmine, lane);
			MM_WAVE_SYNC();
			double av[4];
#pragma unroll
			for (int rb = 0; rb < 4; rb++) av[rb] = pread[16*rb];
			MM_WAVE_SYNC();
			if (k0 + 16 < n) { mm_load_cf(cf, tab, k0 + 16); B.load(k0 + 16, n, bnxt); }
#pragma unroll
			for (int q = 0; q < 4; q++)
#pragma unroll
				for (int rb = 0; rb < 4; rb++) {
					const double aq = q == 0 ? av[rb] : pread[q*MMS_PSTRIDE + 16*rb];
#pragma unroll
					for (int g = 0; g < NG; g++) acc[g][rb] = mm_mfma(aq, bcur[g][q], acc[g][rb]);
				}
			MM_WAVE_SYNC();
#pragma unroll
			for (int g = 0; g < NG; g++)
#pragma unroll
				for (int q = 0; q < 4; q++) bcur[g][q] = bnxt[g][q];
		}
	}
	Sys::template store<NG>(a, m, bb, pbase, PXS_FRESH_INT(lane), acc);
	PXS_COUNT(0, ntile*(NG*256L + 32L) + (wave_alive ? (long)kw*2 : 0L));
}

typedef void (*LegKernel)(const LegK);
static inline bool leg_mm_lds_optin(std::initializer_list<LegKernel> ks) {
	for (LegKernel k : ks) (void)hipFuncSetAttribute((const void*)k, hipFuncAttributeMaxDynamicSharedMemorySize, 160*1024 - 256);
	return true;
}
static inline void leg_launch(LegKernel k, bool analysis, int ng, dim3 grid, hipStream_t st, const LegK& a) {
	const int W = analysis && ng ? MM_WAVES : 1;
	const size_t lds = ng ? (analysis ? mm_ana_lds(ng, MM_WAVES) : mm_syn_lds()) : analysis ? sizeof(double)*LEG_RED_DOUBLES : 0;
	hipLaunchKernelGGL(k, grid, dim3(64*W), lds, st, a);
}
void launch_leg_s0(bool analysis, int ng, int K, dim3 grid, hipStream_t st, const LegK& a);
void launch_leg_spin(bool analysis, int ng, int K, dim3 grid, hipStream_t st, const LegK& a);

}
```

pixell_amd/csrc/sht.hip:

```cpp
#include "sht_plan.hpp"
#include <cmath>
#include <algorithm>

static const char* const ROUTE_NAMES[] = {"direct", "via-cc", "via-cc-unfused", "via-cc-unfused-h", "ring-weights", "cc-weights", "chain", "unfused"};

Route::Scratch Route::scratch(const pxs_plan* p, int nb) const {
	Scratch s; const size_t nct = (size_t)nb*nc, nm = (size_t)p->mmax + 1, c16 = sizeof(double2);
	s.leg = c16*nct*nm*ld_leg_alloc; s.leg2 = c16*nct*nm*ld_leg2; s.h = c16*nct*nr_h*ld_h;
	if (to_map) s.almt = sizeof(double)*4*(tb->nrows + 4)*nb; else s.mom = sizeof(double)*4*std::max<long>(tb->nrows, 1)*nb;
	if (theta_fused && !line) FftChain::theta_scratch(theta, form->tp, (int)nm, (int)nct, s.c1, s.c2);
	if (reserve_chain) p->chain->ring_scratch(p->nring, (int)nct, !to_map, s.r1, p->mmax);
	return s;
}

namespace {

void plan_common(pxs_plan* p, int lmax, int mmax, const uint64_t* mstart, int64_t lstride, int device) {
	PXS_REQUIRE(lmax >= 0 && mmax >= 0 && mmax <= lmax, "need 0 <= mmax <= lmax");
	PXS_REQUIRE(mstart != nullptr, "mstart is required");
	PXS_HIP(hipSetDevice(device));
	p->device = device; p->lmax = lmax; p->mmax = mmax; p->lstride = lstride;
	std::vector<uint64_t> ms(mstart, mstart+mmax+1);
	p->d_mstart = upload(ms);
	p->fc = &fft_context(device);
	{
		size_t fr = 0, tot = 0;
		if (hipMemGetInfo(&fr, &tot) == hipSuccess && fr > 0) p->wk.part_budget = std::min<size_t>(size_t(2) << 30, std::max<size_t>(fr/8, size_t(256) << 20));
		env_budget("PXS_PART_GB", 30, p->wk.part_budget);
		{ const char* d = getenv("PXS_DETERMINISTIC"); p->wk.deterministic = d && atoi(d) != 0; }
	}
	env_budget("PXS_RESAMPLE_MB", 20, p->resample_chunk_bytes);
	{ const char* e = getenv("PXS_ANALYSIS"); if (e) { const std::string v(e); p->ana_weights = v == "weights" ? 1 : (v == "ducc0" ? 2 : (v == "interpolant" ? 0 : p->ana_weights)); } }
	if (p->general) return;
	std::string why;
	if (!FftContext::supported(p->nphi, &why)) throw Error(PXS_ERR_UNSUPPORTED, why);
	std::vector<double2> ph(mmax+1);
	for (int m = 0; m <= mmax; m++) { LDb a = (LDb)m*(LDb)p->phi0; ph[m] = make_double2((double)cosl(a), (double)(-sinl(a))); }
	p->phase = upload(ph);
	p->chain.reset(new FftChain(p->fc));
	p->chain_rings = 2L*mmax < p->nphi && p->chain->plan_rings(p->nphi);
	if (getenv("PXS_CHAIN_VERBOSE")) fprintf(stderr, "[pxsht] ring chain nphi=%d mmax=%d: %s\n", p->nphi, mmax, p->chain_rings ? p->chain->describe().c_str() : "off");
}

void setup_resampling(pxs_plan* p) {
	ThetaTables& t = p->th; AnaForm &ai = p->ana_interp, &af = p->ana_fine;
	af.fine = true;
	if (p->nfull == 0) p->nfull = p->nring;
	GridInfo gi = grid_info(p->geometry, p->nfull);
	t.N = gi.N; t.mir_c = gi.c;
	const int lmax = p->lmax;
	t.Ncc = FftContext::good_size(std::max<long>(2L*lmax + 2, 4));
	if (t.Ncc & 1) t.Ncc = FftContext::good_size(t.Ncc + 1);
	while (t.Ncc & 1) t.Ncc = FftContext::good_size(t.Ncc + 1);
	{
		const long nd = FftChain::ducc_ncc(lmax);
		if (nd >= 4 && FftContext::supported(nd) && FftContext::supported(2*nd)) t.Ncc = nd;
	}
	ai.M = FftContext::good_size(t.N + 2L*lmax + 2);
	if (p->chain_rings) {
		ai.tp = FftChain::plan_theta(t.N, lmax);
		if (ai.tp.ok) { t.Ncc = ai.tp.Ncc; ai.M = ai.tp.M; }
		if (getenv("PXS_CHAIN_VERBOSE")) fprintf(stderr, "[pxsht] theta chain N=%ld lmax=%d: ok=%d g=%ld bN=%ld g2=%ld (M=%ld) ac=%ld (Ncc=%ld) | syn gs=%ld bs=%ld aNs=%ld\n",
			t.N, lmax, (int)ai.tp.ok, ai.tp.g, ai.tp.bN, ai.tp.g2, ai.tp.M, ai.tp.ac, ai.tp.Ncc, ai.tp.gs, ai.tp.bs, ai.tp.aNs);
	}
	t.ncc = (int)(t.Ncc/2 + 1);
	std::string why;
	if (!FftContext::supported(t.N, &why)) throw Error(PXS_ERR_UNSUPPORTED, why);
	std::vector<LDb> th(t.ncc);
	for (int j = 0; j < t.ncc; j++) th[j] = 2*PIl*j/t.Ncc;
	th[t.ncc-1] = PIl;
	p->rs_cc.build(th); p->rs_cc.upload_all();
	const LDb th0 = (LDb)gi.c*PIl/gi.N;
	std::vector<double2> ps(t.N/2 + 1);
	for (long k = 0; k <= t.N/2; k++) { LDb a = (LDb)k*th0; ps[k] = make_double2((double)cosl(a), (double)(-sinl(a))); }
	t.ph_shift = upload(ps);
	{ std::vector<double2> pu(ps.size()); for (size_t k = 0; k < ps.size(); k++) pu[k] = make_double2(ps[k].x, -ps[k].y); t.ph_up = upload(pu); }
	{ const long rings = p->band ? 2L*p->rs_map.npairs : p->nring;
	  p->syn_via_cc = rings > t.ncc + t.ncc/4;
	  p->syn_via_cc0 = rings > t.ncc + t.ncc/2; }
	const long Ks = lmax + t.N/2;
	PXS_REQUIRE(2*Ks < ai.M, "internal: fine grid too small");
	std::vector<double2> spec(ai.M, make_double2(0, 0));
	for (long q = 0; q <= Ks; q++) { double s = abs_sin_coef(q); spec[q].x = s; if (q > 0) spec[ai.M - q].x = s; }
	DevBuf dspec = upload(spec);
	ai.sigma.alloc(sizeof(double2)*ai.M);
	FftDims d;
	FftLoad ld; ld.ptr = dspec.p; FftStore st; st.ptr = ai.sigma.p;
	p->fc->exec(nullptr, ai.M, false, d, ld, st);
	PXS_HIP(hipStreamSynchronize(nullptr));
	std::vector<double2> w(t.ncc);
	for (int j = 0; j < t.ncc; j++) {
		LDb e = (j == 0 || j == t.ncc-1) ? 1 : 2;
		w[j] = make_double2((double)((PIl/p->nphi)*(2*PIl/t.Ncc)*e/((LDb)t.N*(LDb)ai.M)), 0.0);
	}
	ai.wcc = upload(w);
	{
		std::vector<double2> wh(w); for (int j = 1; j + 1 < t.ncc; j++) wh[j].x *= 0.5;
		ai.whalf = upload(wh); }
	{
		std::vector<double2> wa(t.ncc);
		for (int j = 0; j < t.ncc; j++) wa[j] = make_double2(((j == 0 || j == t.ncc-1) ? 0.5 : 1.0)/(double)t.Ncc, 0.0);
		t.wadj = upload(wa); }
	if (FftContext::supported(2*t.Ncc)) {
		if (ai.tp.ok && FftChain::sub_ok_theta(2*ai.tp.ac)) { af.tp = ai.tp; af.tp.g2 = 2*ai.tp.ac; af.tp.M = 2*t.Ncc; } else af.tp.ok = false;
		const long Mf = af.M = 2*t.Ncc; const int nf = (int)(Mf/2 + 1);
		const std::vector<double> gw = grid_weights("CC", nf);
		std::vector<double2> sg(Mf);
		for (long i = 0; i < Mf; i++) {
			const long r = std::min(i, Mf - i);
			const LDb wr = (LDb)gw[r]/(2*PIl)*((r == 0 || r == Mf/2) ? 2 : 1);
			sg[i] = make_double2((double)(wr*(LDb)Mf/(2*PIl)), 0.0);
		}
		af.sigma = upload(sg);
		const double f = (double)ai.M/(double)Mf;
		std::vector<double2> wf(w), whf(w);
		for (int j = 0; j < t.ncc; j++) { wf[j].x *= f; whf[j].x *= (j == 0 || j == t.ncc-1) ? f : 0.5*f; }
		af.wcc = upload(wf); af.whalf = upload(whf);
	}
}

int ncomp_of(int spin, int mode, bool alm_side) {
	if (mode == PXS_MODE_DERIV1) return alm_side ? 1 : 2;
	return spin == 0 ? 1 : 2;
}

void map2leg(pxs_plan* p, hipStream_t st, const Route& r, const MapArg& m, int nb, double2* leg) {
	const int nc = nb*r.nc, ncb = nb > 1 ? r.nc : 0;
	{	StageScope stage(p->prof, st, PXS_STAGE_RING_FFT);
		PXS_REQUIRE(p->chain_rings || (ncb == 0 && (p->general || r.ld_leg == p->nring)), "internal: only the ring chain takes batches and padded rows");
		if (p->general) gen_map2leg(p, st, m, nc, leg, r.ld_leg);
		else if (p->chain_rings) p->chain->map2leg(st, p->map_desc(m, ncb), nc, p->mmax, leg, r.ld_leg, p->phase.as<double2>(), 1.0);
		else unfused_map2leg(p, st, m, nc, leg);
	}
	PXS_HIP(hipGetLastError());
}

void leg2map(pxs_plan* p, hipStream_t st, const Route& r, const double2* leg, long ldleg, const MapArg& m, int nb) {
	const int nc = nb*r.nc, ncb = nb > 1 ? r.nc : 0;
	{	StageScope stage(p->prof, st, PXS_STAGE_RING_FFT);
		PXS_REQUIRE(p->chain_rings || (ncb == 0 && !(p->general && !leg)), "internal: only the ring chain takes batches");
		if (p->general) gen_leg2map(p, st, leg, ldleg, m, nc);
		else {
			if (leg) leg_to_h(p, st, leg, ldleg, r.ld_h, nc);
			const bool full_h = r.nr_h > p->nring;
			if (p->chain_rings) p->chain->h2map(st, p->hbuf.as<double2>() + (full_h ? (size_t)p->row0*r.ld_h : 0), r.ld_h, p->map_desc(m, ncb), nc, p->mmax, full_h ? r.nr_h : 0);
			else unfused_h2map(p, st, m, nc);
		}
	}
	PXS_HIP(hipGetLastError());
}

}

extern "C" {

int pxs_plan_grid2d(pxs_plan** plan, const char* geometry, int ntheta, int nphi, double phi0,
                    int flip_y, int flip_x, int lmax, int mmax, const uint64_t* mstart, int64_t lstride, int device)
{
	PXS_TRY
	PXS_REQUIRE(plan && geometry && ntheta > 0 && nphi > 0, "pxs_plan_grid2d: bad arguments");
	GridInfo gi = grid_info(geometry, ntheta);
	if (!gi.ok) throw Error(PXS_ERR_UNSUPPORTED, std::string("unsupported 2d geometry '") + geometry + "' (supported: CC, F1, MW, MWflip, DH, F2)");
	std::unique_ptr<pxs_plan> p(new pxs_plan());
	p->is_grid = true; p->geometry = geometry; p->nring = ntheta; p->nphi = nphi; p->phi0 = phi0;
	p->ring_stride = flip_y ? -(long)nphi : (long)nphi;
	p->pix_stride = flip_x ? -1 : 1;
	p->ring_off0 = (flip_y ? (long)(ntheta-1)*nphi : 0) + (flip_x ? (long)nphi-1 : 0);
	plan_common(p.get(), lmax, mmax, mstart, lstride, device);
	p->rs_map.build(grid_theta(geometry, ntheta)); p->rs_map.upload_all();
	if (grid_weights_only(geometry)) {
		p->wring = ring_weight_table(geometry, ntheta, nphi);
	} else if (lmax <= grid_maxlmax(geometry, ntheta)) setup_resampling(p.get());
	*plan = p.release();
	PXS_CATCH
}

int pxs_plan_rings(pxs_plan** plan, int nring, const double* theta, const uint64_t* nphi,
                   const double* phi0, const uint64_t* ringstart, int64_t pixstride,
                   int lmax, int mmax, const uint64_t* mstart, int64_t lstride, int device)
{
	PXS_TRY
	PXS_REQUIRE(plan && nring > 0 && theta && nphi && phi0 && ringstart, "pxs_plan_rings: bad arguments");
	std::unique_ptr<pxs_plan> p(new pxs_plan());
	p->is_grid = false; p->nring = nring; p->nphi = (int)nphi[0]; p->phi0 = phi0[0];
	p->ring_off0 = (long)ringstart[0];
	p->ring_stride = nring > 1 ? (long)ringstart[1] - (long)ringstart[0] : (long)nphi[0];
	for (int r = 0; r < nring; r++)
		if ((long)nphi[r] != p->nphi || std::fabs(phi0[r] - phi0[0]) > 1e-13 || (long)ringstart[r] != p->ring_off0 + r*p->ring_stride) p->general = true;
	if (!FftContext::supported(p->nphi)) p->general = true;
	{ const char* e = getenv("PXS_GENERAL_RINGS"); if (e && atoi(e) != 0) p->general = true; }
	p->pix_stride = pixstride;
	plan_common(p.get(), lmax, mmax, mstart, lstride, device);
	if (p->general) p->gen.setup(device, nring, nphi, phi0, ringstart);
	std::vector<LDb> th(nring);
	for (int r = 0; r < nring; r++) th[r] = theta[r];
	p->rs_map.build(th); p->rs_map.upload_all();
	if (!p->general && p->chain_rings && nring >= 2) {
		const LDb d = th[1] - th[0];
		const long n = d > 0 ? (long)llroundl(PIl/d) : 0;
		const long k0 = n > 0 ? (long)llroundl(th[0]*n/PIl - 0.5L) : -1;
		bool ok = n > nring && k0 >= 0 && k0 + nring <= n && lmax <= n - 1 && n < (1L << 30) && FftContext::supported(2*n);
		for (int r = 0; ok && r < nring; r++) ok = fabsl(th[r] - ((LDb)(k0 + r) + 0.5L)*PIl/n) < 1e-11L;
		if (ok) {
			p->band = true; p->geometry = "F1"; p->nfull = (int)n; p->row0 = (int)k0;
			setup_resampling(p.get());
			if (!p->chain_theta()) { p->band = false; p->nfull = 0; p->row0 = 0; p->th.ncc = 0; }
		}
	}
	*plan = p.release();
	PXS_CATCH
}

int pxs_plan_points(pxs_plan** plan, const pxs_plan* g, int64_t npts, const double* d_loc, double epsilon, int device, void* stream)
{
	PXS_TRY
	PXS_REQUIRE(plan && g && npts >= 0 && (d_loc || npts == 0), "pxs_plan_points: bad arguments");
	PXS_REQUIRE(g->is_grid && g->geometry == "CC" && !g->pts && g->phi0 == 0 && g->ring_stride == g->nphi && g->pix_stride == 1,
		"pxs_plan_points: needs an unflipped CC grid plan with phi0 = 0");
	PXS_REQUIRE(g->nring >= g->lmax + 2 && g->nphi % 2 == 0 && g->nphi >= 2*g->mmax + 2, "pxs_plan_points: the CC grid needs ntheta >= lmax + 2 and an even nphi >= 2 mmax + 2");
	PXS_REQUIRE(FftContext::supported(2L*g->nring - 2) && FftContext::supported(g->nphi), "pxs_plan_points: CC grid sizes the FFT engine cannot transform");
	PXS_REQUIRE(epsilon >= 1e-13 && epsilon <= 0.1, "pxs_plan_points: epsilon must lie in [1e-13, 0.1]");
	PXS_REQUIRE(device == g->device, "pxs_plan_points: the grid plan lives on another device");
	PXS_HIP(hipSetDevice(device));
	std::unique_ptr<pxs_plan> p(new pxs_plan());
	p->device = device; p->lmax = g->lmax; p->mmax = g->mmax; p->lstride = g->lstride; p->pgrid = const_cast<pxs_plan*>(g);
	p->pts = points_create(g->nring, g->nphi, g->lmax, g->mmax, device, (long)npts, d_loc, epsilon, (hipStream_t)stream);
	*plan = p.release();
	PXS_CATCH
}

void pxs_plan_destroy(pxs_plan* plan) { delete plan; }

int pxs_plan_option(pxs_plan* p, const char* name, int64_t value) {
	PXS_TRY
	PXS_REQUIRE(p && name, "pxs_plan_option: null argument");
	std::lock_guard<std::mutex> plan_lock(p->call_mu);
	if (p->pts) {
		const std::string n(name);
		PXS_REQUIRE((n == "deterministic" || n == "profile") && (value == 0 || value == 1), "pxs_plan_option: a points plan takes 'deterministic' or 'profile' (0 or 1)");
		if (n == "deterministic") p->wk.deterministic = value != 0;
		else points_profile(p->pts, value != 0);
		return 0;
	}
	if (std::string(name) == "analysis") {
		PXS_REQUIRE(value >= 0 && value <= 2, "pxs_plan_option: analysis takes 0 (interpolant), 1 (weights) or 2 (ducc0)");
		p->ana_weights = (int)value;
	} else if (std::string(name) == "deterministic") {
		PXS_REQUIRE(value == 0 || value == 1, "pxs_plan_option: deterministic takes 0 or 1");
		p->wk.deterministic = value != 0;
	} else if (std::string(name) == "build_tables") {
		PXS_REQUIRE(value >= 0 && value <= p->lmax + 1, "pxs_plan_option: build_tables takes a spin");
		PXS_HIP(hipSetDevice(p->device));
		(void)p->table((int)value);
	} else if (std::string(name) == "leg_max_batch") {
		PXS_REQUIRE(value >= 0 && value <= (1 << 20), "pxs_plan_option: leg_max_batch takes 0 (no bound) or a number of maps");
		p->wk.max_batch = (int)value;
	} else if (std::string(name) == "leg_ana_k") {
		PXS_REQUIRE(value >= 0 && value <= 64, "pxs_plan_option: leg_ana_k takes 0 (the host's rule) or a number of ring pairs per lane");
		p->wk.ana_k = (int)value;
	} else throw Error(PXS_ERR_ARG, std::string("pxs_plan_option: unknown option '") + name + "'");
	PXS_CATCH
}

static const AnaForm& ana_form(const pxs_plan* p) { return p->ana_weights != 0 && p->ana_fine.M > 0 ? p->ana_fine : p->ana_interp; }

static void run_theta(pxs_plan* p, hipStream_t st, const Route& r, int nct, int spin, const double2* wring) {
	const ThetaTables& t = p->th; const AnaForm& f = *r.form;
	const bool to_h = r.theta == TH_FROM_CC || r.theta == TH_TO_CC_ADJ, mid = r.theta == TH_TO_CC || r.theta == TH_TO_CC_ADJ;
	ThetaCall c;
	c.tp = &f.tp; c.nc = nct; c.nm = p->mmax + 1; c.spin = spin; c.lmax = p->lmax; c.mir_c = t.mir_c;
	c.map = (to_h ? p->hbuf : p->leg).as<double2>(); c.ldmap = to_h ? r.ld_h : r.ld_leg; c.nr = to_h ? r.nr_h : r.nr_th;
	c.cc = p->leg2.as<double2>(); c.ldcc = r.ld_leg2; c.ncc = t.ncc;
	c.ph = (r.theta == TH_FROM_CC ? t.ph_up : t.ph_shift).as<double2>();
	if (mid) c.sigma = f.sigma.as<double2>();
	if (r.theta != TH_FROM_CC) c.wcc = (r.theta == TH_TO_CC ? f.wcc : r.theta == TH_TO_CC_ADJ ? f.whalf : t.wadj).as<double2>();
	c.wring = wring;
	if (to_h) { c.tab = p->phase.as<double2>(); c.scale = mid ? 2.0 : 1.0/(double)t.Ncc; }
	p->chain->theta(st, r.theta, c);
}
static Route route_of(const pxs_plan* p, bool analysis, int spin, int mode, bool adjoint, const LegTables* tb);
static Route analysis_route_now(const pxs_plan* p) { return route_of(p, true, 0, PXS_MODE_STANDARD, false, nullptr); }
static std::vector<ChainShape> chain_shapes(const pxs_plan* cp) {
	pxs_plan* p = const_cast<pxs_plan*>(cp);
	std::vector<ChainShape> all, out;
	if (!p->chain || !p->chain_rings) return out;
	std::lock_guard<std::mutex> plan_lock(p->call_mu);
	FftChain::MapDesc md; memset(&md, 0, sizeof(md)); md.dtype = PX_F64; md.cstride = (long)p->nring*p->nphi; md.ring_stride = p->nphi; md.pix_stride = 1; md.nring = p->nring; md.nphi = p->nphi;
	p->chain->dry_begin(&all);
	try {
		for (int which = 0; which < 3; which++) {
			const bool ana = which == 0; const int spin = which == 2 ? 2 : 0;
			const Route r = route_of(p, ana, spin, PXS_MODE_STANDARD, false, nullptr);
			if (!r.reserve_chain) continue;
			if (ana) p->chain->map2leg(nullptr, md, r.nc, p->mmax, nullptr, r.ld_leg, nullptr, 1.0);
			else p->chain->h2map(nullptr, nullptr, r.ld_h, md, r.nc, p->mmax, 0);
			if (r.theta_fused && !r.line) run_theta(p, nullptr, r, r.nc, spin, nullptr);
		}
	} catch (...) { p->chain->dry_end(); throw; }
	p->chain->dry_end();
	for (const ChainShape& c : all) {
		bool seen = false;
		for (const ChainShape& o : out) seen = seen || (o.sid == c.sid && o.na == c.na && o.nb == c.nb && o.T == c.T);
		if (!seen) out.push_back(c);
	}
	return out;
}
int pxs_plan_query(const pxs_plan* p, const char* name, int64_t* value) {
	PXS_TRY
	PXS_REQUIRE(name && value, "pxs_plan_query: null argument");
	const std::string n(name);
	if (n.compare(0, 7, "passes_") == 0) {
		std::string seam = n.substr(7); int which = 0;
		static const char* const sufs[3] = {"_first", "_prev", "_last"};
		for (int i = 0; i < 3 && !which; i++) {
			const size_t k = strlen(sufs[i]);
			if (seam.size() > k && seam.compare(seam.size() - k, k, sufs[i]) == 0) { seam.resize(seam.size() - k); which = i + 1; }
		}
		const PassLog* l = nullptr;
		if (seam == "fft") { int dev = p ? p->device : 0; if (!p) PXS_HIP(hipGetDevice(&dev)); l = &fft_context(dev).pass_lines; }
		else {
			PXS_REQUIRE(p && !p->pts, "pxs_plan_query: the passes of this seam belong to a grid or ring plan");
			if (seam == "batch") l = &p->pass_batch; else if (seam == "resample") l = &p->pass_resample;
			else if (seam == "leg_m") l = &p->wk.pass_m; else if (seam == "leg_valu") l = &p->wk.pass_valu; else if (seam == "leg_mm") l = &p->wk.pass_mm;
			else if ((seam == "theta" || seam == "ring") && p->chain) l = seam == "theta" ? &p->chain->pass_theta : &p->chain->pass_ring;
		}
		if (!l) throw Error(PXS_ERR_ARG, std::string("pxs_plan_query: unknown name '") + name + "'");
		*value = which == 0 ? l->n : which == 1 ? l->first : which == 2 ? l->prev : l->last;
		return 0;
	}
	PXS_REQUIRE(p, "pxs_plan_query: null argument");
	if (p->pts) *value = points_query(p->pts, n);
	else if (n == "analysis_form") { const Route r = analysis_route_now(p); *value = (r.kind == R_RING_WEIGHTS || r.kind == R_CC_WEIGHTS) ? 1 : (r.form->fine ? 2 : 0); }
	else if (n == "leg_ana_k") *value = p->wk.last_ana_k;
	else if (n == "ncc_circle") *value = p->th.ncc > 0 ? p->th.Ncc : 0;
	else if (n == "ducc_ncc_circle") *value = FftChain::ducc_ncc(p->lmax);
	else if (n == "theta_line") *value = analysis_route_now(p).line ? 1 : 0;
	else if (n == "chain_stages" || n == "chain_static") {
		int64_t k = 0;
		for (const ChainShape& c : chain_shapes(p)) {
			if (getenv("PXS_CHAIN_VERBOSE")) fprintf(stderr, "[pxsht] plan stage %d: na=%d nb=%d T=%d static %d\n", c.sid, c.na, c.nb, c.T, c.is_static ? 1 : 0);
			k += (n == "chain_stages" || c.is_static) ? 1 : 0;
		}
		*value = k;
	}
	else if (n == "chain_static_table") *value = p->chain ? p->chain->static_check(0) : 0;
	else throw Error(PXS_ERR_ARG, std::string("pxs_plan_query: unknown name '") + name + "'");
	PXS_CATCH
}

int pxs_plan_info(const pxs_plan* p, int* nsyn, int* nana, int64_t* scratch) {
	if (!p) return PXS_ERR_ARG;
	if (nsyn) *nsyn = route_of(p, false, 2, PXS_MODE_STANDARD, false, nullptr).rs->nring;
	if (nana) *nana = p->th.ncc > 0 ? p->th.ncc : p->nring;
	if (scratch) *scratch = (int64_t)(p->leg.bytes + p->leg2.bytes + p->hbuf.bytes + p->b1.bytes + p->b2.bytes + p->wk.almt.bytes + p->wk.part.bytes + p->wk.mom.bytes);
	return 0;
}

int pxs_debug_theta_plan(int64_t N, int lmax, int64_t* out) {
	const ThetaPlan t = FftChain::plan_theta(N, lmax);
	const int64_t v[10] = {t.ok, t.g, t.bN, t.g2, t.M, t.ac, t.Ncc, t.gs, t.bs, t.aNs};
	for (int i = 0; i < 10; i++) out[i] = v[i];
	return 0;
}

int pxs_debug_chain(pxs_plan* p, int kind, int nc, int spin, int reps, double* ms) {
	PXS_TRY
	PXS_REQUIRE(p && ms && nc >= 1 && reps >= 1 && kind >= 0 && kind <= 4, "pxs_debug_chain: bad arguments");
	PXS_REQUIRE(p->chain_rings && (kind < 2 || p->chain_theta()), "pxs_debug_chain: the plan has no fused chain for this stage");
	PXS_HIP(hipSetDevice(p->device));
	std::lock_guard<std::mutex> plan_lock(p->call_mu);
	PlanUse use(p, nullptr);
	const size_t nm = (size_t)p->mmax + 1, nr = (size_t)p->nring, c16 = sizeof(double2);
	const long ldm = FftChain::pad8(p->nring), ldc = p->ld_cc(), ldh = p->ld_h();
	DevBuf dmap;
	if (kind < 2) { dmap.alloc(sizeof(double)*(size_t)nc*nr*p->nphi); PXS_HIP(hipMemset(dmap.p, 0, dmap.bytes)); }
	p->leg.ensure(c16*nc*nm*ldm); p->leg2.ensure(c16*nc*nm*std::max<long>(ldc, 8)); p->hbuf.ensure(c16*nc*nr*ldh);
	PXS_HIP(hipMemset(p->leg.p, 0, p->leg.bytes)); PXS_HIP(hipMemset(p->leg2.p, 0, p->leg2.bytes)); PXS_HIP(hipMemset(p->hbuf.p, 0, p->hbuf.bytes));
	hipStream_t st = nullptr;
	Route r;
	r.ld_leg = ldm; r.nr_th = p->nring; r.ld_leg2 = ldc; r.ld_h = ldh; r.nr_h = p->nring;
	r.theta = kind == 2 ? TH_TO_CC : (kind == 3 ? TH_FROM_CC : TH_FROM_CC_ADJ);
	r.form = kind == 2 && ana_form(p).tp.ok ? &ana_form(p) : &p->ana_interp;
	auto run = [&]() {
		const FftChain::MapDesc md = p->map_desc(MapArg{dmap.p, PX_F64, (long)nr*p->nphi, 0});
		if (kind == 0) p->chain->map2leg(st, md, nc, p->mmax, p->leg.as<double2>(), ldm, p->phase.as<double2>(), 1.0);
		else if (kind == 1) p->chain->h2map(st, p->hbuf.as<double2>(), ldh, md, nc, p->mmax);
		else run_theta(p, st, r, nc, spin, nullptr);
	};
	run(); PXS_HIP(hipStreamSynchronize(st));
	hipEvent_t e0, e1; PXS_HIP(hipEventCreate(&e0)); PXS_HIP(hipEventCreate(&e1));
	PXS_HIP(hipEventRecord(e0, st));
	for (int i = 0; i < reps; i++) run();
	PXS_HIP(hipEventRecord(e1, st)); PXS_HIP(hipEventSynchronize(e1));
	float t = 0; PXS_HIP(hipEventElapsedTime(&t, e0, e1));
	(void)hipEventDestroy(e0); (void)hipEventDestroy(e1);
	*ms = (double)t/reps;
	PXS_CATCH
}

int pxs_profile(pxs_plan* p, int enable) {
	PXS_TRY
	PXS_REQUIRE(p, "pxs_profile: null plan");
	p->prof.enabled = enable != 0;
	if (enable && !p->wk.count.p) { PXS_HIP(hipSetDevice(p->device)); p->wk.count.alloc(2*1024*sizeof(double)); PXS_HIP(hipMemset(p->wk.count.p, 0, p->wk.count.bytes)); }
	p->wk.count_on = enable != 0;
	PXS_CATCH
}

int pxs_profile_flops(pxs_plan* p, double* flops, int reset) {
	PXS_TRY
	PXS_REQUIRE(p && flops, "pxs_profile_flops: null argument");
	flops[0] = flops[1] = 0;
	if (!p->wk.count.p) return 0;
	PXS_HIP(hipSetDevice(p->device));
	PXS_HIP(hipDeviceSynchronize());
	std::vector<double> c(p->wk.count.bytes/sizeof(double)); PXS_HIP(hipMemcpy(c.data(), p->wk.count.p, p->wk.count.bytes, hipMemcpyDeviceToHost));
	for (size_t i = 0; i + 1 < c.size(); i += 2) { flops[0] += c[i]*128.0; flops[1] += c[i+1]*128.0; }
	if (reset) PXS_HIP(hipMemset(p->wk.count.p, 0, p->wk.count.bytes));
	PXS_CATCH
}

int pxs_profile_read(pxs_plan* p, double* ms, int* counts, int reset) {
	PXS_TRY
	PXS_REQUIRE(p && ms && counts, "pxs_profile_read: null argument");
	p->prof.read(ms, counts, PXS_NSTAGE, reset != 0);
	PXS_CATCH
}

static Route route_of(const pxs_plan* p, bool analysis, int spin, int mode, bool adjoint, const LegTables* tb) {
	Route r;
	const int nr = p->nring;
	const bool th = p->chain_theta();
	const long ldm = p->ld_map(), ldc = p->ld_cc(), ldh = p->ld_h();
	r.to_map = analysis ? adjoint : !adjoint; r.tb = tb;
	r.nc = analysis ? (spin == 0 ? 1 : 2) : ncomp_of(spin, mode, false); r.deriv1 = mode == PXS_MODE_DERIV1;
	r.rs = &p->rs_map; r.nr_th = nr; r.form = &p->ana_interp;
	auto use_h = [&](int rows) { r.nr_h = rows; r.ld_h = ldh; };
	if (!analysis) {
		const bool cc = (p->is_grid || (p->band && th)) && (spin == 0 ? p->syn_via_cc0 : p->syn_via_cc) && p->th.ncc > 0;
		r.ld_leg = r.ld_leg_alloc = ldm;
		if (!cc || (adjoint && !th)) { r.kind = R_DIRECT; if (!adjoint && !p->general) use_h(nr); }
		else {
			r.rs = &p->rs_cc; r.ld_leg2 = ldc; r.nr_th = p->band ? p->nfull : nr;
			if (adjoint) { r.kind = R_VIA_CC; r.theta = TH_FROM_CC_ADJ; r.ld_leg = r.ld_leg_alloc = p->band ? FftChain::pad8(p->nfull) : ldm; }
			else if (th) { r.kind = R_VIA_CC; r.theta = TH_FROM_CC; use_h(r.nr_th); r.ld_leg = 0; }
			else { r.kind = !p->chain_rings ? R_VIA_CC_UNFUSED_H : R_VIA_CC_UNFUSED; r.theta = TH_FROM_CC; use_h(nr); r.ld_leg = nr; }
		}
	} else if (p->wring.p) { r.kind = R_RING_WEIGHTS; }
	else if ((p->ana_weights == 1 || (p->ana_weights == 2 && p->geometry == "CC")) && (long)nr >= 2L*p->lmax + 2)
		r.kind = (th && p->th.ncc > 0) ? R_CC_WEIGHTS : R_RING_WEIGHTS;
	else {
		r.form = &ana_form(p);
		auto adj_ana_fused = [] { const char* e = getenv("PXS_ADJ_ANA_FUSED"); return e ? atoi(e) != 0 : true; };
		r.kind = (th && (r.form->fine ? r.form->tp.ok : (!adjoint || adj_ana_fused()))) ? R_CHAIN : R_UNFUSED;
	}
	if (analysis) {
		if (r.kind == R_RING_WEIGHTS) { r.ld_leg = ldm; if (adjoint) use_h(nr); }
		else {
			r.rs = &p->rs_cc; r.ld_leg2 = r.kind == R_UNFUSED ? p->th.ncc : ldc;
			if (!adjoint || r.kind == R_UNFUSED) r.ld_leg = r.kind == R_UNFUSED ? nr : ldm;
			if (adjoint) use_h(nr);
			r.theta = r.kind == R_CC_WEIGHTS ? (adjoint ? TH_FROM_CC : TH_FROM_CC_ADJ) : (adjoint ? TH_TO_CC_ADJ : TH_TO_CC);
		}
		r.ld_leg_alloc = r.ld_leg;
	}
	const bool unfused = r.kind == R_VIA_CC_UNFUSED || r.kind == R_VIA_CC_UNFUSED_H || r.kind == R_UNFUSED;
	r.batched = !unfused;
	r.theta_fused = r.theta != TH_NONE && !unfused;
	r.line = r.theta_fused && r.theta <= TH_FROM_CC_ADJ && FftChain::line_takes(r.form->tp, r.theta == TH_TO_CC);
	r.reserve_chain = p->chain_rings && r.kind != R_UNFUSED;
	return r;
}

static const double2* ring_weights(pxs_plan* p) {
	if (p->wring.p) return p->wring.as<double2>();
	if (!p->th.wgrid.p) p->th.wgrid = ring_weight_table(p->geometry, p->nring, p->nphi);
	return p->th.wgrid.as<double2>();
}
static const double2* ring_weights_ext(pxs_plan* p) {
	const double2* w = ring_weights(p);
	if (p->geometry == "F1") return w;
	if (!p->th.wgrid_ext.p) {
		std::vector<double2> wd(p->nring);
		PXS_HIP(hipMemcpy(wd.data(), w, sizeof(double2)*p->nring, hipMemcpyDeviceToHost));
		for (int r = 0; r < p->nring; r++) if (self_mirrored(r, p->th.mir_c, p->th.N)) wd[r].x *= 2;
		p->th.wgrid_ext = upload(wd);
	}
	return p->th.wgrid_ext.as<double2>();
}

static const double2* unit_weights_ext(pxs_plan* p) {
	if (p->geometry == "F1" || p->band) return nullptr;
	if (!p->th.wunit_ext.p) {
		std::vector<double2> wd(p->nring, make_double2(1, 0));
		for (int r = 0; r < p->nring; r++) if (self_mirrored(r, p->th.mir_c, p->th.N)) wd[r].x = 2;
		p->th.wunit_ext = upload(wd);
	}
	return p->th.wunit_ext.as<double2>();
}

static void run_core(pxs_plan* p, const Route& r, int spin, int nb, const AlmArg& alm, const MapArg& map, hipStream_t st)
{
	const int nct = nb*r.nc, nr = p->nring, nm = p->mmax + 1;
	double2* leg = p->leg.as<double2>();
	switch (r.kind) {
	case R_VIA_CC_UNFUSED: case R_VIA_CC_UNFUSED_H: {
		PXS_REQUIRE(nb == 1, "internal: batched call on an unfused path");
		const bool to_h = r.kind == R_VIA_CC_UNFUSED_H;
		p->leg_syn(st, r, alm, 1);
		resample_from_cc(p, st, p->leg2.as<double2>(), leg, r.nc, spin, to_h ? p->hbuf.as<double2>() : nullptr);
		leg2map(p, st, r, to_h ? nullptr : leg, r.ld_leg, map, 1);
		return; }
	case R_UNFUSED:
		PXS_REQUIRE(nb == 1, "internal: batched call on an unfused path");
		if (r.to_map) {
			p->leg_syn(st, r, alm, 1);
			resample_to_cc_adjoint(p, st, p->leg2.as<double2>(), leg, r.nc, spin, *r.form);
			leg2map(p, st, r, leg, r.ld_leg, map, 1);
		} else {
			map2leg(p, st, r, map, 1, leg);
			resample_to_cc(p, st, leg, p->leg2.as<double2>(), r.nc, spin, *r.form);
			p->leg_ana(st, r, alm, 1);
		}
		return;
	default: break;
	}
	const double2* wleg = r.kind == R_RING_WEIGHTS ? ring_weights(p) : nullptr;
	const double2* wth = r.kind == R_CC_WEIGHTS ? (r.to_map ? ring_weights(p) : ring_weights_ext(p)) : (r.kind == R_VIA_CC && !r.to_map ? unit_weights_ext(p) : nullptr);
	auto weigh = [&] { if (wleg) scale_leg_rings(st, leg, (long)nct*nm, nr, r.ld_leg, wleg); };
	auto theta = [&] { if (r.theta != TH_NONE) { StageScope stage(p->prof, st, PXS_STAGE_RESAMPLE); run_theta(p, st, r, nct, spin, wth); } };
	if (r.to_map) {
		p->leg_syn(st, r, alm, nb);
		weigh();
		theta();
		leg2map(p, st, r, r.theta != TH_NONE ? nullptr : leg, r.ld_leg, map, nb);
	} else {
		if (r.nr_th > nr) {
			PXS_HIP(hipMemsetAsync(p->leg.p, 0, sizeof(double2)*(size_t)nct*nm*r.ld_leg, st));
			leg += p->row0;
		}
		map2leg(p, st, r, map, nb, leg);
		weigh();
		theta();
		p->leg_ana(st, r, alm, nb);
	}
}

static void reserve_call(pxs_plan* p, const Route& r, int nb) {
	const Route::Scratch s = r.scratch(p, nb);
	p->wk.almt.ensure(s.almt); p->wk.mom.ensure(s.mom);
	p->leg.ensure(s.leg); p->leg2.ensure(s.leg2); p->hbuf.ensure(s.h);
	if (r.reserve_chain) p->chain->reserve(std::max(s.c1, s.r1), s.c2);
}

static int batch_chunk(const pxs_plan* p, int nbatch, int ncm) {
	if (nbatch <= 1 || !p->chain_rings) return 1;
	const size_t per_map = sizeof(double2)*(size_t)ncm*((size_t)(p->mmax+1)*(p->nring + (p->th.ncc > 0 ? p->th.ncc : 0))*2 + (size_t)p->nring*p->nphi);
	size_t budget_env = 0; env_budget("PXS_BATCH_GB", 30, budget_env);
	size_t budget = budget_env ? budget_env : (size_t)64 << 30;
	if (!budget_env) {
		size_t fr = 0, tot = 0;
		const size_t held = p->leg.bytes + p->leg2.bytes + p->hbuf.bytes + (p->chain ? p->chain->scratch_bytes() : 0);
		if (hipMemGetInfo(&fr, &tot) == hipSuccess && fr > 0) budget = std::min(budget, std::max<size_t>((size_t)4 << 30, held + (size_t)(0.4*(double)fr)));
	}
	const int cap = (int)std::max<size_t>(1, std::min<size_t>((size_t)nbatch, budget/std::max<size_t>(per_map, 1)));
	if (ncm == 1 && cap >= 8 && nbatch > cap) {
		const int cap8 = cap & ~7, npass = (nbatch + cap8 - 1)/cap8;
		return std::min(cap8, (((nbatch + npass - 1)/npass + 7)/8)*8);
	}
	const int npass = (nbatch + cap - 1)/cap;
	return (nbatch + npass - 1)/npass;
}

static void run_call(pxs_plan* p, bool analysis, int spin, int mode, int adjoint, int nbatch, const AlmArg& alm, const MapArg& map, hipStream_t st) {
	const Route r = route_of(p, analysis, spin, mode, adjoint != 0, &p->table(spin));
	const int chunk = r.batched ? batch_chunk(p, nbatch, r.nc) : 1;
	if (getenv("PXS_CHAIN_VERBOSE")) fprintf(stderr, "[pxsht] %s route %s, adjoint %d, spin %d, analysis option %d, %d maps in passes of %d\n", analysis ? "analysis" : "synthesis", ROUTE_NAMES[r.kind], adjoint, spin, p->ana_weights, nbatch, chunk);
	reserve_call(p, r, std::min(chunk, nbatch));
	p->pass_batch.begin(); p->pass_resample.begin(); p->wk.pass_m.begin(); p->wk.pass_valu.begin(); p->wk.pass_mm.begin();
	if (p->chain) { p->chain->pass_theta.begin(); p->chain->pass_ring.begin(); }
	for (int b0 = 0; b0 < nbatch; b0 += chunk) {
		p->pass_batch.add(std::min(chunk, nbatch - b0));
		run_core(p, r, spin, std::min(chunk, nbatch - b0), alm.from(b0), map.from(b0), st);
	}
}

int pxs_synthesis(pxs_plan* p, int spin, int mode, int adjoint, int nbatch,
                  void* alm, int alm_dtype, int64_t alm_cstride, int64_t alm_bstride,
                  void* map, int map_dtype, int64_t map_cstride, int64_t map_bstride, void* stream)
{
	PXS_TRY
	PXS_REQUIRE(p && alm && map, "pxs_synthesis: null argument");
	std::lock_guard<std::mutex> plan_lock(p->call_mu);
	PXS_REQUIRE(spin >= 0 && spin <= p->lmax + 1, "pxs_synthesis: bad spin");
	PXS_REQUIRE(mode == PXS_MODE_STANDARD || (mode == PXS_MODE_DERIV1 && spin == 1), "DERIV1 needs spin 1");
	PXS_REQUIRE(map_dtype == PX_F32 || map_dtype == PX_F64, "map must be float32 or float64");
	PXS_REQUIRE(nbatch >= 1, "pxs_synthesis: nbatch must be >= 1");
	PXS_HIP(hipSetDevice(p->device));
	hipStream_t st = (hipStream_t)stream;
	PlanUse use(p, st);
	const AlmArg a{alm, alm_dtype, (long)alm_cstride, (long)alm_bstride}; const MapArg m{map, map_dtype, (long)map_cstride, (long)map_bstride};
	if (p->pts) points_run(p->pts, p->pgrid, spin, mode, adjoint, nbatch, a, m, st);
	else run_call(p, false, spin, mode, adjoint, nbatch, a, m, st);
	PXS_CATCH
}

int pxs_analysis(pxs_plan* p, int spin, int adjoint, int nbatch,
                 void* map, int map_dtype, int64_t map_cstride, int64_t map_bstride,
                 void* alm, int alm_dtype, int64_t alm_cstride, int64_t alm_bstride, void* stream)
{
	PXS_TRY
	PXS_REQUIRE(p && alm && map, "pxs_analysis: null argument");
	std::lock_guard<std::mutex> plan_lock(p->call_mu);
	PXS_REQUIRE(p->is_grid, "pxs_analysis needs a grid2d plan");
	PXS_REQUIRE(map_dtype == PX_F32 || map_dtype == PX_F64, "map must be float32 or float64");
	PXS_REQUIRE(nbatch >= 1, "pxs_analysis: nbatch must be >= 1");
	if (p->lmax > grid_maxlmax(p->geometry, p->nring)) throw Error(PXS_ERR_ARG, "too few rings for analysis up to requested lmax");
	PXS_HIP(hipSetDevice(p->device));
	hipStream_t st = (hipStream_t)stream;
	PlanUse use(p, st);
	run_call(p, true, spin, PXS_MODE_STANDARD, adjoint, nbatch, AlmArg{alm, alm_dtype, (long)alm_cstride, (long)alm_bstride}, MapArg{map, map_dtype, (long)map_cstride, (long)map_bstride}, st);
	PXS_CATCH
}

}
```

pixell_amd/sht.py:

```python
import ctypes, os, contextlib, threading
import numpy as np
from . import _lib, _arrays as A
from ._arrays import device_index, current_stream

_tls = threading.local()
def _pipe(): return getattr(_tls, "pipe", None)
@contextlib.contextmanager
def host_pipeline(inputs=(), outputs=()):
	from . import hostio
	if _pipe() is not None or _lib.is_hostsim() or not any(hostio.eligible(a) for a in list(inputs)+list(outputs)):
		yield; return
	_tls.pipe = hostio.Pipeline(); _tls.pipe.prefetch(inputs)
	try: yield
	finally:
		p = _tls.pipe; _tls.pipe = None; p.close()

class _Buf:
	def __init__(self, arr, writeback=False, overwrite=False):
		self.arr = arr; self.writeback = writeback; self.tmp = None; self.keep = None; self.slab = False
		if A.is_tensor(arr):
			A.require_gpu(arr)
			if not arr.is_contiguous():
				if writeback: raise ValueError("output tensors must be contiguous")
				arr = arr.contiguous()
			self.keep = arr; self.ptr = arr.data_ptr()
		else:
			if _lib.is_hostsim():
				if arr.flags.c_contiguous and arr.dtype.isnative: self.keep = arr
				else: self.keep = np.ascontiguousarray(arr); self.tmp = self.keep
				self.ptr = self.keep.ctypes.data
			else:
				torch = A.torch()
				from . import hostio
				pipe = _pipe(); got = pipe.take(arr) if pipe is not None else None
				self.slab = hostio.eligible(arr)
				if got is not None:
					self.tmp, ev = got; torch.cuda.current_stream().wait_event(ev)
					self.tmp.record_stream(torch.cuda.current_stream())
				elif self.slab and writeback and overwrite:
					self.tmp = A.empty(arr.shape, arr.dtype)
				elif self.slab:
					self.tmp, ev = hostio.upload(arr); torch.cuda.current_stream().wait_event(ev)
				else: self.tmp = A.put(arr)
				self.ptr = self.tmp.data_ptr()
	def finish(self):
		if not self.writeback or self.tmp is None: return
		if _lib.is_hostsim(): self.arr[...] = self.tmp
		elif self.slab:
			from . import hostio
			ev = A.torch().cuda.Event(); ev.record()
			pipe = _pipe()
			if pipe is not None: pipe.writeback(self.tmp, self.arr, ev)
			else: hostio.download(self.tmp, self.arr, after=ev)
		else: self.arr[...] = A.host(self.tmp)

class Plan:
	def __init__(self, handle):
		self.handle = handle; self.lock = threading.RLock()
		self._det_default = int(os.environ.get("PXS_DETERMINISTIC", "0") not in ("", "0"))
	def __del__(self):
		try:
			if self.handle: _lib.load().pxs_plan_destroy(self.handle); self.handle = None
		except Exception: pass
	def profile(self, enable=True):
		_lib.check(_lib.load().pxs_profile(self.handle, int(bool(enable))))
	def profile_read(self, reset=True):
		ms = (ctypes.c_double*4)(); cnt = (ctypes.c_int*4)()
		_lib.check(_lib.load().pxs_profile_read(self.handle, ms, cnt, int(bool(reset))))
		names = ["leg_syn", "leg_ana", "ring_fft", "resample"]
		return {n: (ms[i], cnt[i]) for i, n in enumerate(names)}
	def profile_flops(self, reset=True):
		f = (ctypes.c_double*2)()
		_lib.check(_lib.load().pxs_profile_flops(self.handle, f, int(bool(reset))))
		return f[0], f[1]
	def set_option(self, name, value):
		_lib.check(_lib.load().pxs_plan_option(self.handle, name.encode(), int(value)))
	def query(self, name):
		v = ctypes.c_int64()
		_lib.check(_lib.load().pxs_plan_query(self.handle, name.encode(), ctypes.byref(v)))
		return int(v.value)
	def passes(self, seam):
		return _passes(self.handle, seam)
	def info(self):
		a, b, c = ctypes.c_int(), ctypes.c_int(), ctypes.c_int64()
		_lib.check(_lib.load().pxs_plan_info(self.handle, ctypes.byref(a), ctypes.byref(b), ctypes.byref(c)))
		return dict(nring_syn=a.value, nring_ana=b.value, scratch_bytes=c.value)

def _passes(handle, seam):
	out = {}
	for key, suffix in (("n", ""), ("first", "_first"), ("prev", "_prev"), ("last", "_last")):
		v = ctypes.c_int64()
		_lib.check(_lib.load().pxs_plan_query(handle, ("passes_" + seam + suffix).encode(), ctypes.byref(v)))
		out[key] = int(v.value)
	return out
def fft_passes():
	return _passes(None, "fft")

class _PlanCache:
	def __init__(self):
		import collections
		self.d = collections.OrderedDict()
		self.cap = max(1, int(os.environ.get("PIXELL_AMD_MAX_PLANS", "4")))
	def get(self, key):
		p = self.d.get(key)
		if p is not None: self.d.move_to_end(key)
		return p
	def __setitem__(self, key, plan):
		self.d[key] = plan; self.d.move_to_end(key)
		while len(self.d) > self.cap: self.d.popitem(last=False)
	def clear(self): self.d.clear()
	def __len__(self): return len(self.d)
_plans = _PlanCache()
def clear_plans(release=False):
	_plans.clear()
	if release: memory(release=True)

def memory(release=False):
	import gc; gc.collect()
	st = (ctypes.c_double*6)()
	_lib.check(_lib.load().pxs_memory(int(bool(release)), st))
	return dict(malloc_ms=st[0], malloc_calls=int(st[1]), malloc_bytes=int(st[2]), arena_hits=int(st[3]), arena_bytes=int(st[4]), live_bytes=int(st[5]))

class PlanPin:
	def __init__(self): self.plans = {}
	def __enter__(self):
		if not hasattr(_tls, "pins"): _tls.pins = []
		_tls.pins.append(self); return self
	def __exit__(self, *exc): _tls.pins.pop(); return False
	def clear(self): self.plans.clear()
	def __len__(self): return len(self.plans)

def _cached_plan(key, make):
	pins = getattr(_tls, "pins", None)
	pin = pins[-1] if pins else None
	p = pin.plans.get(key) if pin is not None else None
	if p is None: p = _plans.get(key)
	if p is None:
		p = Plan(make())
		if pin is None: _plans[key] = p
	if pin is not None: pin.plans[key] = p
	return p

_deterministic = None
def set_deterministic(on=True):
	global _deterministic
	_deterministic = None if on is None else bool(on)
def _apply_mode(plan):
	want = _deterministic
	if want is None and getattr(plan, "_det", None) is not None:
		plan.set_option("deterministic", plan._det_default); plan._det = None
	elif want is not None and getattr(plan, "_det", None) != want:
		plan.set_option("deterministic", int(want)); plan._det = want
	return plan

def tri_mstart(lmax, mmax=None):
	if mmax is None: mmax = lmax
	m = np.arange(mmax+1, dtype=np.int64)
	return (m*(2*lmax+1-m)//2).astype(np.uint64)

def grid_plan(geometry, ntheta, nphi, phi0, flip, lmax, mmax, mstart, lstride=1):
	ms = np.ascontiguousarray(np.asarray(mstart)[:mmax+1], dtype=np.uint64)
	key = ("g", geometry, int(ntheta), int(nphi), float(phi0), bool(flip[0]), bool(flip[1]), int(lmax), int(mmax), ms.tobytes(), int(lstride), device_index())
	def make():
		h = ctypes.c_void_p()
		_lib.check(_lib.load().pxs_plan_grid2d(ctypes.byref(h), geometry.encode(), int(ntheta), int(nphi), float(phi0),
			int(bool(flip[0])), int(bool(flip[1])), int(lmax), int(mmax), ms.ctypes.data, int(lstride), device_index()))
		return h
	return _cached_plan(key, make)

def ring_plan(theta, nphi, phi0, ringstart, lmax, mmax, mstart, lstride=1, pixstride=1):
	th = np.ascontiguousarray(theta, dtype=np.float64); nph = np.ascontiguousarray(nphi, dtype=np.uint64)
	p0 = np.ascontiguousarray(phi0, dtype=np.float64); rs = np.ascontiguousarray(ringstart, dtype=np.uint64)
	ms = np.ascontiguousarray(np.asarray(mstart)[:mmax+1], dtype=np.uint64)
	key = ("r", th.tobytes(), nph.tobytes(), p0.tobytes(), rs.tobytes(), int(pixstride), int(lmax), int(mmax), ms.tobytes(), int(lstride), device_index())
	def make():
		h = ctypes.c_void_p()
		_lib.check(_lib.load().pxs_plan_rings(ctypes.byref(h), len(th), th.ctypes.data, nph.ctypes.data, p0.ctypes.data, rs.ctypes.data,
			int(pixstride), int(lmax), int(mmax), ms.ctypes.data, int(lstride), device_index()))
		return h
	return _cached_plan(key, make)

def _ncomp(spin, mode):
	if mode == "DERIV1": return 1, 2
	return (1, 1) if spin == 0 else (2, 2)

def _check_pair(alm, map, spin, mode, pixdims):
	nca, ncm = _ncomp(spin, mode)
	if mode not in ("STANDARD", "DERIV1"): raise ValueError("unknown mode '%s'" % str(mode))
	if alm.ndim == 3 and map.ndim == 2+pixdims:
		if alm.shape[0] != map.shape[0]: raise ValueError("batched call: alm and map disagree on the batch size")
		alm, map = alm[0], map[0]
	if alm.ndim != 2 or alm.shape[0] != nca: raise ValueError("alm must have shape [%d,nelem] for spin %d mode %s" % (nca, spin, mode))
	if map.ndim != 1+pixdims or map.shape[0] != ncm: raise ValueError("map must have %d components" % ncm)
	ad, md = A.np_dtype(alm), A.np_dtype(map)
	if ad not in (np.complex64, np.complex128) or md not in (np.float32, np.float64): raise TypeError("alm must be complex, map real")
	return ad, md

class _View:
	def __init__(self, arr, inner_ndim, batched, writeback, overwrite=False):
		self.buf = None
		if A.is_tensor(arr) and (arr.is_cuda or _lib.is_hostsim()):
			st = list(arr.stride()); sh = list(arr.shape)
			inner_ok = all(st[-k] == int(np.prod(sh[len(sh)-k+1:], dtype=np.int64)) for k in range(1, inner_ndim+1))
			if inner_ok:
				self.keep = arr; self.ptr = arr.data_ptr()
				self.cstride = st[-inner_ndim-1]; self.bstride = st[0] if batched else 0
				return
		self.buf = _Buf(arr, writeback=writeback, overwrite=overwrite); self.ptr = self.buf.ptr
		inner = int(np.prod(arr.shape[arr.ndim-inner_ndim:], dtype=np.int64))
		self.cstride = inner; self.bstride = inner*arr.shape[-inner_ndim-1] if batched else 0
	def finish(self):
		if self.buf is not None: self.buf.finish()

def _run_syn(plan, alm, map, spin, mode, adjoint, map_overwrite=False):
	ad, md = A.np_dtype(alm), A.np_dtype(map)
	batched = alm.ndim == 3
	nb = alm.shape[0] if batched else 1
	av = _View(alm, 1, batched, bool(adjoint)); mv = _View(map, map.ndim-(2 if batched else 1), batched, not adjoint, overwrite=map_overwrite and not adjoint)
	with plan.lock:
		_apply_mode(plan)
		_lib.check(_lib.load().pxs_synthesis(plan.handle, int(spin), 1 if mode == "DERIV1" else 0, int(bool(adjoint)), int(nb),
			av.ptr, A.DT[ad], av.cstride, av.bstride, mv.ptr, A.DT[md], mv.cstride, mv.bstride, current_stream()))
	av.finish(); mv.finish()

ANALYSIS_MODES = {"ducc0": 2, "interpolant": 0, "weights": 1}
def _analysis_mode(analysis):
	if analysis is None: analysis = os.environ.get("PIXELL_AMD_ANALYSIS", "ducc0")
	if analysis not in ANALYSIS_MODES: raise ValueError("analysis must be 'ducc0', 'interpolant' or 'weights', not %r" % (analysis,))
	return ANALYSIS_MODES[analysis]

def analysis_form(geometry, ntheta, nphi, lmax, mmax=None, mstart=None, phi0=0.0, lstride=1, flip=(False, False), analysis=None):
	if mmax is None: mmax = lmax
	if mstart is None: mstart = tri_mstart(lmax, mmax)
	plan = grid_plan(geometry, ntheta, nphi, phi0, flip, lmax, mmax, mstart, lstride)
	plan.set_option("analysis", _analysis_mode(analysis))
	return dict(form={0: "interpolant", 1: "weights", 2: "ducc0"}[plan.query("analysis_form")], ncc_circle=plan.query("ncc_circle"), ducc_ncc_circle=plan.query("ducc_ncc_circle"))

def _run_ana(plan, map, alm, spin, adjoint, analysis=None, alm_dense=False):
	ad, md = A.np_dtype(alm), A.np_dtype(map)
	batched = alm.ndim == 3
	nb = alm.shape[0] if batched else 1
	av = _View(alm, 1, batched, not adjoint, overwrite=alm_dense and not adjoint); mv = _View(map, map.ndim-(2 if batched else 1), batched, bool(adjoint), overwrite=bool(adjoint))
	with plan.lock:
		_apply_mode(plan)
		plan.set_option("analysis", _analysis_mode(analysis))
		_lib.check(_lib.load().pxs_analysis(plan.handle, int(spin), int(bool(adjoint)), int(nb), mv.ptr, A.DT[md], mv.cstride, mv.bstride,
			av.ptr, A.DT[ad], av.cstride, av.bstride, current_stream()))
	av.finish(); mv.finish()

def _grid_args(alm, map, spin, lmax, mmax, mstart, geometry, phi0, lstride, mode, flip):
	_check_pair(alm, map, spin, mode, 2)
	if mmax is None: mmax = lmax
	if mstart is None: mstart = tri_mstart(lmax, mmax)
	nt, nph = map.shape[-2:]
	return grid_plan(geometry, nt, nph, phi0, flip, lmax, mmax, mstart, lstride)

def synthesis_2d(*, alm, map, spin, lmax, geometry, mmax=None, mstart=None, phi0=0.0, nthreads=0, lstride=1, mode="STANDARD", flip=(False, False), return_plan=False):
	plan = _grid_args(alm, map, spin, lmax, mmax, mstart, geometry, phi0, lstride, mode, flip)
	_run_syn(plan, alm, map, spin, mode, False, map_overwrite=True)
	return plan if return_plan else map

def adjoint_synthesis_2d(*, alm, map, spin, lmax, geometry, mmax=None, mstart=None, phi0=0.0, nthreads=0, lstride=1, mode="STANDARD", flip=(False, False), return_plan=False):
	plan = _grid_args(alm, map, spin, lmax, mmax, mstart, geometry, phi0, lstride, mode, flip)
	_run_syn(plan, alm, map, spin, mode, True)
	return plan if return_plan else alm

def analysis_2d(*, alm, map, spin, lmax, geometry, mmax=None, mstart=None, phi0=0.0, nthreads=0, lstride=1, flip=(False, False), return_plan=False, analysis=None):
	plan = _grid_args(alm, map, spin, lmax, mmax, mstart, geometry, phi0, lstride, "STANDARD", flip)
	dense = lstride == 1 and (mmax is None or mmax == lmax) and alm.shape[-1] == (lmax+1)*(lmax+2)//2 and (mstart is None or int(np.asarray(mstart)[-1]) + lmax + 1 == alm.shape[-1])
	_run_ana(plan, map, alm, spin, False, analysis, alm_dense=dense)
	return plan if return_plan else alm

def adjoint_analysis_2d(*, alm, map, spin, lmax, geometry, mmax=None, mstart=None, phi0=0.0, nthreads=0, lstride=1, flip=(False, False), return_plan=False, analysis=None):
	plan = _grid_args(alm, map, spin, lmax, mmax, mstart, geometry, phi0, lstride, "STANDARD", flip)
	_run_ana(plan, map, alm, spin, True, analysis)
	return plan if return_plan else map

def _ring_args(alm, map, theta, nphi, phi0, ringstart, lmax, mmax, mstart, spin, lstride, pixstride, mode):
	if mmax is None: mmax = lmax
	if mstart is None: mstart = tri_mstart(lmax, mmax)
	return ring_plan(theta, nphi, phi0, ringstart, lmax, mmax, mstart, lstride, pixstride), mmax, mstart

def synthesis(*, alm, theta, nphi, phi0, ringstart, lmax, mmax=None, mstart=None, spin=0, map=None, lstride=1, pixstride=1, nthreads=0, mode="STANDARD"):
	plan, mmax, mstart = _ring_args(alm, map, theta, nphi, phi0, ringstart, lmax, mmax, mstart, spin, lstride, pixstride, mode)
	nca, ncm = _ncomp(spin, mode)
	if map is None:
		rs_ = np.asarray(ringstart).astype(np.int64); last_ = rs_+(np.asarray(nphi).astype(np.int64)-1)*pixstride
		npix = int(max(rs_.max(), last_.max())+1)
		rdt = np.float32 if A.np_dtype(alm) == np.complex64 else np.float64
		map = A.zeros((ncm, npix), rdt, like=alm)
	_check_pair(alm, map, spin, mode, 1)
	_run_syn(plan, alm, map, spin, mode, False)
	synthesis.last_plan = plan
	return map

def adjoint_synthesis(*, map, theta, nphi, phi0, ringstart, lmax, mmax=None, mstart=None, spin=0, alm=None, lstride=1, pixstride=1, nthreads=0, mode="STANDARD"):
	plan, mmax, mstart = _ring_args(alm, map, theta, nphi, phi0, ringstart, lmax, mmax, mstart, spin, lstride, pixstride, mode)
	nca, ncm = _ncomp(spin, mode)
	if alm is None:
		nelem = int(np.max(np.asarray(mstart).astype(np.int64))+lmax*lstride+1)
		cdt = np.complex64 if A.np_dtype(map) == np.float32 else np.complex128
		alm = A.zeros((nca, nelem), cdt, like=map)
	_check_pair(alm, map, spin, mode, 1)
	_run_syn(plan, alm, map, spin, mode, True)
	adjoint_synthesis.last_plan = plan
	return alm

EPS_MIN, EPS_MAX = 1e-13, 0.1

def points_grid_shape(lmax, mmax):
	g = _lib.load().pxf_fft_good_size
	return int(g(lmax+1))+1, 2*int(g(mmax+1))

def _loc_device(loc):
	tens = A.is_tensor(loc); xp = A.torch() if tens else np
	loc = loc.to(xp.float64).contiguous() if tens else np.ascontiguousarray(loc, dtype=np.float64)
	if loc.ndim != 2 or loc.shape[1] != 2: raise ValueError("loc must have shape [npts, 2]")
	if loc.shape[0] and not bool(((loc[:, 0] >= 0) & (loc[:, 0] <= np.pi) & xp.isfinite(loc[:, 1])).all()):
		raise ValueError("loc: theta must lie in [0, pi] and phi be finite")
	if _lib.is_hostsim() or (tens and loc.is_cuda): return loc, loc.shape[0]
	return A.to_gpu(loc), loc.shape[0]

def points_plan(loc, lmax, mmax=None, mstart=None, lstride=1, epsilon=1e-10):
	if mmax is None: mmax = lmax
	if mstart is None: mstart = tri_mstart(lmax, mmax)
	epsilon = float(epsilon)
	if not (EPS_MIN <= epsilon <= EPS_MAX): raise ValueError("epsilon must lie in [%g, %g], got %g" % (EPS_MIN, EPS_MAX, epsilon))
	nt, nph = points_grid_shape(lmax, mmax)
	grid = grid_plan("CC", nt, nph, 0.0, (False, False), lmax, mmax, mstart, lstride)
	dloc, npts = _loc_device(loc)
	h = ctypes.c_void_p()
	_lib.check(_lib.load().pxs_plan_points(ctypes.byref(h), grid.handle, int(npts), A.ptr(dloc) if npts else None, epsilon, device_index(), current_stream()))
	p = Plan(h); p.grid = grid; p.npts = int(npts)
	return p

def points_profile(plan, enable=True):
	plan.set_option("profile", int(bool(enable)))

def points_profile_read(plan):
	out = {k: plan.query("stage_us_"+k)*1e-3 for k in ("cc_sht", "fft", "grid", "interp", "spread")}
	out["plan"] = plan.query("plan_us")*1e-3
	return out

def _default_eps(epsilon, map_dtype):
	if epsilon is not None: return epsilon
	return 1e-6 if np.dtype(map_dtype) == np.float32 else 1e-10

def _run_points(plan, alm, map, spin, mode, adjoint):
	with plan.grid.lock:
		_apply_mode(plan.grid)
		_run_syn(plan, alm, map, spin, mode, adjoint, map_overwrite=True)

def _use_plan(plan, loc, lmax, mmax, mstart, lstride, epsilon, map_dtype):
	if plan is not None:
		if plan.npts != int(loc.shape[0]): raise ValueError("plan was made for %d points, loc has %d" % (plan.npts, int(loc.shape[0])))
		return plan
	return points_plan(loc, lmax, mmax, mstart, lstride, _default_eps(epsilon, map_dtype))

def synthesis_general(*, alm, loc, spin, lmax, mmax=None, mstart=None, lstride=1, epsilon=None, mode="STANDARD", map=None, nthreads=0, plan=None):
	nca, ncm = _ncomp(spin, mode)
	if mode not in ("STANDARD", "DERIV1"): raise ValueError("unknown mode '%s'" % str(mode))
	npts = int(loc.shape[0])
	if map is None:
		rdt = np.float32 if A.np_dtype(alm) == np.complex64 else np.float64
		shape = tuple(alm.shape[:-2])+(ncm, npts)
		map = A.zeros(shape, rdt, like=alm)
	_check_pair(alm, map, spin, mode, 1)
	if map.shape[-1] != npts: raise ValueError("map has %d points, loc %d" % (map.shape[-1], npts))
	plan = _use_plan(plan, loc, lmax, mmax, mstart, lstride, epsilon, A.np_dtype(map))
	if npts == 0: return map
	_run_points(plan, alm, map, spin, mode, False)
	return map

def adjoint_synthesis_general(*, map, loc, spin, lmax, mmax=None, mstart=None, lstride=1, epsilon=None, mode="STANDARD", alm=None, nthreads=0, plan=None):
	nca, ncm = _ncomp(spin, mode)
	if mode not in ("STANDARD", "DERIV1"): raise ValueError("unknown mode '%s'" % str(mode))
	if mmax is None: mmax = lmax
	if mstart is None: mstart = tri_mstart(lmax, mmax)
	npts = int(loc.shape[0])
	if alm is None:
		nelem = int(np.max(np.asarray(mstart).astype(np.int64))+lmax*lstride+1)
		cdt = np.complex64 if A.np_dtype(map) == np.float32 else np.complex128
		shape = tuple(map.shape[:-2])+(nca, nelem)
		alm = A.zeros(shape, cdt, like=map)
	_check_pair(alm, map, spin, mode, 1)
	if map.shape[-1] != npts: raise ValueError("map has %d points, loc %d" % (map.shape[-1], npts))
	plan = _use_plan(plan, loc, lmax, mmax, mstart, lstride, epsilon, A.np_dtype(map))
	if npts == 0:
		alm[...] = 0
		return alm
	_run_points(plan, alm, map, spin, mode, True)
	return alm

_gridweights_cache = {}
def rotate_alm(alm, lmax, psi, theta, phi, nthreads=1):
	from . import almops
	return almops.rotate_alm(alm, lmax, psi, theta, phi, inplace=False)

def get_gridweights(geometry, ntheta):
	key = (str(geometry), int(ntheta))
	out = _gridweights_cache.get(key)
	if out is None:
		out = np.zeros(int(ntheta), np.float64)
		_lib.check(_lib.load().pxs_gridweights(geometry.encode(), int(ntheta), out.ctypes.data))
		if len(_gridweights_cache) >= 8: _gridweights_cache.pop(next(iter(_gridweights_cache)))
		_gridweights_cache[key] = out
	return out.copy()

def grid_maxlmax(geometry, ntheta):
	return int(_lib.load().pxs_grid_maxlmax(geometry.encode(), int(ntheta)))
```

Before: 3.703.

## Stage analysis Legendre kernels to accumulate only rings that have become live

The spin-0 and spin analysis kernels now move through compile-time stages, and each stage adds one more ring slot to the moment accumulation. A slot joins once its Legendre values become live, detected by a warp vote or read from per-slot start indices stored in the seed buffer. Before this, every slot accumulated data FMAs from the first live step even when its own recurrence values were still negligible. The change adds code size, extra branch checks every four steps, and a larger profiling counter layout that tracks executed flops.

New measurement: 3.742, median of 6. +1.0%, better.

```diff
diff --git a/pixell_amd/csrc/leg_s0.hip b/pixell_amd/csrc/leg_s0.hip
--- a/pixell_amd/csrc/leg_s0.hip
+++ b/pixell_amd/csrc/leg_s0.hip
@@ -28,9 +28,13 @@
 		if (a.seed_mode == 1) { \
 			double* sd = a.seed_d + ((long)m*a.nwave + wv)*(2*K*64); int* si = a.seed_i + ((long)m*a.nwave + wv)*((K+1)*64); \
 			_Pragma("unroll") for (int s = 0; s < K; s++) { sd[s*64 + lane] = lam1[s]; sd[(K+s)*64 + lane] = lam2[s]; si[s*64 + lane] = sc[s]; } \
-			if (lane == 0) si[K*64] = k; \
-		} \
-	}
+			if (lane == 0) si[K*64] = k; else if (lane <= K) si[K*64 + lane] = LEG_NEVER; \
+		} \
+	}
+#define S0_BLOCK_STARTS(c) ((k & 3) == 0 && (a.seed_mode == 2 ? k >= knext : __any(leg_live_upto<c>(lam2, sc))))
+#define S0_SEED_TAIL (a.seed_i + ((long)m*a.nwave + wv)*((K+1)*64) + K*64)
+#define S0_BLOCK_BEGIN(c) { PXS_COUNT_BLOCK(DIR, (long)(nk - k)*4); if (a.seed_mode == 1 && lane == (c) + 1) S0_SEED_TAIL[(c) + 1] = k; }
+#define S0_NEXT_START(c) if (a.seed_mode == 2) knext = PXS_UNIFORM_INT(S0_SEED_TAIL[(c) + 1]);
 
 #define S0_SYN_PAIR(c0, c1, a0, a1) S0_SYN_PAIR_C(c0.a, polar ? c0.c : c0.b, c1.a, polar ? c1.c : c1.b, a0, a1)
 #define S0_SYN_PAIR_C(ca0, cb0, ca1, cb1, a0, a1) { \
@@ -142,11 +146,11 @@
 	PXS_VCOPY(vb1, polar ? c1.c : c1.b); \
 	double t0 = 0, t1 = 0, t2 = 0, t3 = 0, u0 = 0, u1 = 0, u2 = 0, u3 = 0; \
 	_Pragma("unroll") for (int s = 0; s < K; s++) { \
-		t0 = fma(lam2[s], d1r[s], t0); t1 = fma(lam2[s], d1i[s], t1); t2 = fma(lam2[s], d2r[s], t2); t3 = fma(lam2[s], d2i[s], t3); \
+		if (s >= SLO) { t0 = fma(lam2[s], d1r[s], t0); t1 = fma(lam2[s], d1i[s], t1); t2 = fma(lam2[s], d2r[s], t2); t3 = fma(lam2[s], d2i[s], t3); } \
 		lam1[s] = fma(fma(c0.a, csq[s], vb0), lam2[s], lam1[s]); \
 	} \
 	_Pragma("unroll") for (int s = 0; s < K; s++) { \
-		u0 = fma(lam1[s], d1r[s], u0); u1 = fma(lam1[s], d1i[s], u1); u2 = fma(lam1[s], d2r[s], u2); u3 = fma(lam1[s], d2i[s], u3); \
+		if (s >= SLO) { u0 = fma(lam1[s], d1r[s], u0); u1 = fma(lam1[s], d1i[s], u1); u2 = fma(lam1[s], d2r[s], u2); u3 = fma(lam1[s], d2i[s], u3); } \
 		lam2[s] = fma(fma(c1.a, csq[s], vb1), lam1[s], lam2[s]); \
 	} \
 	 \
@@ -158,7 +162,7 @@
 #define S0_ANA_STEP_C(ca, cb, LA, LB, T0, T1, T2, T3) { \
 	PXS_VCOPY(vb, cb); \
 	_Pragma("unroll") for (int s = 0; s < K; s++) { \
-		T0 = fma(LA[s], d1r[s], T0); T1 = fma(LA[s], d1i[s], T1); T2 = fma(LA[s], d2r[s], T2); T3 = fma(LA[s], d2i[s], T3); \
+		if (s >= SLO) { T0 = fma(LA[s], d1r[s], T0); T1 = fma(LA[s], d1i[s], T1); T2 = fma(LA[s], d2r[s], T2); T3 = fma(LA[s], d2i[s], T3); } \
 		LB[s] = fma(fma(ca, csq[s], vb), LA[s], LB[s]); \
 	} }
 #define S0_ANA_PAIR_D(ca0, cb0, ca1, cb1, kfirst, NEXT) { \
@@ -174,6 +178,60 @@
 	LEG_RED_PUT(kk, t0, t1, t2, t3) \
 	LEG_RED_PUT(kk+1, u0, u1, u2, u3) \
 	kk += 2; }
+
+#define S0_ANA_STAGE(NB) if constexpr ((NB) <= K) { if (nb == (NB)) { \
+	constexpr int SLO = K - (NB); \
+	bool more = false; \
+	if (!inC) { \
+	while (k + 1 < nk) { \
+		if constexpr ((NB) < K) if (k < nk && S0_BLOCK_STARTS(SLO - 1)) { more = true; break; } \
+		bool pend = false; \
+		_Pragma("unroll") for (int s = 0; s < K; s++) pend |= (sc[s] < 0); \
+		if (!__any(pend)) break; \
+		for (int it = 0; it < 2 && k + 1 < nk; it++, k += 2) { \
+			const double4_t c0 = LDC(coef, k), c1 = LDC(coef, k+1); \
+			S0_ANA_PAIR(c0, c1) \
+		} \
+		_Pragma("unroll") for (int s = 0; s < K; s++) \
+			if (sc[s] < 0 && fabs(lam2[s]) > SC_BIG) { \
+				lam1[s] *= SC_SMALL; lam2[s] *= SC_SMALL; \
+				if (++sc[s] == 0 && s >= SLO) load_data(s); \
+			} \
+	} \
+	if (!more) { \
+		n = LDC2(cf, k); f = LDC2(cf, k+1); \
+		PXS_ROWS_DRAIN(); \
+		n.a1 = n.a0; n.b1 = n.b0;       \
+		inC = 1; \
+	} } \
+	if (!more) { \
+		for (;;) {       \
+			if constexpr ((NB) < K) if (k < nk && S0_BLOCK_STARTS(SLO - 1)) { more = true; break; } \
+			if (!(k + 3 < nk)) break; \
+			S0_ANA_PAIR_D(n.a1, n.b1, f.a0, f.b0, k, n = LDC2(cf, k+3)) \
+			S0_ANA_PAIR_D(f.a1, f.b1, n.a0, n.b0, k+2, f = LDC2(cf, k+5)) \
+			k += 4; \
+		} \
+	} \
+	if (!more) { \
+		slo = SLO; \
+		nb = K + 1; \
+	} else if constexpr ((NB) < K) { S0_BLOCK_BEGIN(SLO - 1) if (sc[SLO - 1] == 0) load_data(SLO - 1); if constexpr ((NB) + 1 < K) { S0_NEXT_START(SLO - 2) } nb = (NB) + 1; } \
+} }
+#define S0_ANA_TAIL { const int SLO = slo; \
+		if (k + 1 < nk) { \
+			S0_ANA_PAIR_D(n.a1, n.b1, f.a0, f.b0, k, (void)0) \
+			k += 2; \
+		} \
+		PXS_ROWS_DRAIN(); \
+		if (kk == LEG_FSTEPS) { leg_flush(red, pout + 4*kbase, lane, LEG_FSTEPS, a.atomic); kk = 0; kbase = k; } \
+		if (k < nk) { \
+			double t0 = 0, t1 = 0, t2 = 0, t3 = 0; \
+			_Pragma("unroll") for (int s = 0; s < K; s++) if (s >= SLO) { t0 = fma(lam2[s], d1r[s], t0); t1 = fma(lam2[s], d1i[s], t1); t2 = fma(lam2[s], d2r[s], t2); t3 = fma(lam2[s], d2i[s], t3); } \
+			LEG_RED_PUT(kk, t0, t1, t2, t3) \
+			kk++; \
+		} }
+
 
 template<int K> __global__ __launch_bounds__(64) void leg_ana_s0(const LegK a)
 {
@@ -216,49 +274,19 @@
 	int k = 0;
 	S0_SEEDED_PHASE_A
 	k = PXS_UNIFORM_INT(k); coef = (const double4_t*)PXS_UNIFORM_LONG((long)coef);
-	PXS_COUNT(1, (long)(nk - k)*K*6 + (a.seed_mode != 2 ? (long)k*K*2 : 0L));
+	constexpr int DIR = 1;
+	PXS_COUNT2(DIR, (long)(nk - k)*K*2 + (a.seed_mode != 2 ? (long)k*K*2 : 0L), (long)(nk - k)*4, K);
+	int knext = LEG_NEVER;
+	if constexpr (K > 1) { S0_NEXT_START(K - 2) }
 	if (lane == 0 && !a.atomic) a.first[wv*a.nmc + (m - a.m0)] = k + 1;
-#pragma unroll
-	for (int s = 0; s < K; s++) if (sc[s] == 0) load_data(s);
+	if (sc[K - 1] == 0) load_data(K - 1);
 	int kk = 0, kbase = k;
-	while (k + 1 < nk) {
-		bool pend = false;
-#pragma unroll
-		for (int s = 0; s < K; s++) pend |= (sc[s] < 0);
-		if (!__any(pend)) break;
-		for (int it = 0; it < 2 && k + 1 < nk; it++, k += 2) {
-			const double4_t c0 = LDC(coef, k), c1 = LDC(coef, k+1);
-			S0_ANA_PAIR(c0, c1)
-		}
-#pragma unroll
-		for (int s = 0; s < K; s++)
-			if (sc[s] < 0 && fabs(lam2[s]) > SC_BIG) {
-				lam1[s] *= SC_SMALL; lam2[s] *= SC_SMALL;
-				if (++sc[s] == 0) load_data(s);
-			}
-	}
 	const double2* __restrict__ cf = (const double2*)PXS_UNIFORM_LONG((long)((polar ? a.coef2p : a.coef2) + row0));
-	coef2x2_t n = LDC2(cf, k), f = LDC2(cf, k+1);
-	PXS_ROWS_DRAIN();
-	n.a1 = n.a0; n.b1 = n.b0;
-	while (k + 3 < nk) {
-		S0_ANA_PAIR_D(n.a1, n.b1, f.a0, f.b0, k, n = LDC2(cf, k+3))
-		S0_ANA_PAIR_D(f.a1, f.b1, n.a0, n.b0, k+2, f = LDC2(cf, k+5))
-		k += 4;
-	}
-	if (k + 1 < nk) {
-		S0_ANA_PAIR_D(n.a1, n.b1, f.a0, f.b0, k, (void)0)
-		k += 2;
-	}
-	PXS_ROWS_DRAIN();
-	if (kk == LEG_FSTEPS) { leg_flush(red, pout + 4*kbase, lane, LEG_FSTEPS, a.atomic); kk = 0; kbase = k; }
-	if (k < nk) {
-		double t0 = 0, t1 = 0, t2 = 0, t3 = 0;
-#pragma unroll
-		for (int s = 0; s < K; s++) { t0 = fma(lam2[s], d1r[s], t0); t1 = fma(lam2[s], d1i[s], t1); t2 = fma(lam2[s], d2r[s], t2); t3 = fma(lam2[s], d2i[s], t3); }
-		LEG_RED_PUT(kk, t0, t1, t2, t3)
-		kk++;
-	}
+	coef2x2_t n, f;
+	int nb = 1, inC = 0, slo = 0;
+	S0_ANA_STAGE(1) S0_ANA_STAGE(2) S0_ANA_STAGE(3) S0_ANA_STAGE(4) S0_ANA_STAGE(5) S0_ANA_STAGE(6) S0_ANA_STAGE(7) S0_ANA_STAGE(8)
+	static_assert(K <= 8, "leg_ana_s0: one S0_ANA_STAGE per block (K = 12 takes four more and was measured with them: profiles/README.md, \"Block starts\")");
+	S0_ANA_TAIL
 	if (kk > 0) leg_flush(red, pout + 4*kbase, lane, kk, a.atomic);
 }
 
diff --git a/pixell_amd/csrc/leg_spin.hip b/pixell_amd/csrc/leg_spin.hip
--- a/pixell_amd/csrc/leg_spin.hip
+++ b/pixell_amd/csrc/leg_spin.hip
@@ -79,9 +79,13 @@
 			_Pragma("unroll") for (int s = 0; s < K; s++) { \
 				sd[s*64 + lane] = S.gp1[s]; sd[(K+s)*64 + lane] = S.gp2[s]; sd[(2*K+s)*64 + lane] = S.gm1[s]; sd[(3*K+s)*64 + lane] = S.gm2[s]; \
 				si[s*64 + lane] = S.scp[s]; si[(K+s)*64 + lane] = S.scm[s]; } \
-			if (lane == 0) si[2*K*64] = j; \
-		} \
-	}
+			if (lane == 0) si[2*K*64] = j; else if (lane <= K) si[2*K*64 + lane] = LEG_NEVER; \
+		} \
+	}
+#define SPIN_BLOCK_STARTS(c) ((j & 3) == 0 && (a.seed_mode == 2 ? j >= knext : __any(leg_live_upto<c>(S.gp2, S.scp) || leg_live_upto<c>(S.gm2, S.scm))))
+#define SPIN_SEED_TAIL (a.seed_i + ((long)m*a.nwave + wv)*((2*K+1)*64) + 2*K*64)
+#define SPIN_BLOCK_BEGIN(c) { PXS_COUNT_BLOCK(DIR, (long)(nl - j)*8); if (a.seed_mode == 1 && lane == (c) + 1) SPIN_SEED_TAIL[(c) + 1] = j; }
+#define SPIN_NEXT_START(c) if (a.seed_mode == 2) knext = PXS_UNIFORM_INT(SPIN_SEED_TAIL[(c) + 1]);
 
 struct spin_rows_t { double4_t r0, r1; };
 __device__ __forceinline__ spin_rows_t spin_rows(const double4_t* coef, long i) { spin_rows_t r; r.r0 = LDC(coef, i); r.r1 = LDC(coef, i+1); return r; }
@@ -222,10 +226,12 @@
 		PXS_VCOPY(v1, c1); PXS_VCOPY(v2, c2); \
 		_Pragma("unroll") for (int s = 0; s < K; s++) { \
 			const double gp = S.gp2[s], gm = S.gm2[s]; \
-			t0 = fma(gp, tpnr[s], t0); t0 = fma(gm, tpsr[s], t0); \
-			t1 = fma(gp, tpni[s], t1); t1 = fma(gm, tpsi[s], t1); \
-			t2 = fma(gm, tmnr[s], t2); t2 = fma(gp, tmsr[s], t2); \
-			t3 = fma(gm, tmni[s], t3); t3 = fma(gp, tmsi[s], t3); \
+			if (s >= SLO) { \
+				t0 = fma(gp, tpnr[s], t0); t0 = fma(gm, tpsr[s], t0); \
+				t1 = fma(gp, tpni[s], t1); t1 = fma(gm, tpsi[s], t1); \
+				t2 = fma(gm, tmnr[s], t2); t2 = fma(gp, tmsr[s], t2); \
+				t3 = fma(gm, tmni[s], t3); t3 = fma(gp, tmsi[s], t3); \
+			} \
 			S.gp1[s] = fma(fma(ca, S.x[s], v1), gp, -S.gp1[s]); S.gm1[s] = fma(fma(ca, S.x[s], v2), gm, -S.gm1[s]); \
 		} \
 	} \
@@ -234,10 +240,12 @@
 		PXS_VCOPY(v1, c1); PXS_VCOPY(v2, c2); \
 		_Pragma("unroll") for (int s = 0; s < K; s++) { \
 			const double gp = S.gp1[s], gm = S.gm1[s]; \
-			u0 = fma(gp, tpnr[s], u0); u0 = fma(-gm, tpsr[s], u0); \
-			u1 = fma(gp, tpni[s], u1); u1 = fma(-gm, tpsi[s], u1); \
-			u2 = fma(gm, tmnr[s], u2); u2 = fma(-gp, tmsr[s], u2); \
-			u3 = fma(gm, tmni[s], u3); u3 = fma(-gp, tmsi[s], u3); \
+			if (s >= SLO) { \
+				u0 = fma(gp, tpnr[s], u0); u0 = fma(-gm, tpsr[s], u0); \
+				u1 = fma(gp, tpni[s], u1); u1 = fma(-gm, tpsi[s], u1); \
+				u2 = fma(gm, tmnr[s], u2); u2 = fma(-gp, tmsr[s], u2); \
+				u3 = fma(gm, tmni[s], u3); u3 = fma(-gp, tmsi[s], u3); \
+			} \
 			S.gp2[s] = fma(fma(ca, S.x[s], v1), gp, -S.gp2[s]); S.gm2[s] = fma(fma(ca, S.x[s], v2), gm, -S.gm2[s]); \
 		} \
 	} \
@@ -251,20 +259,24 @@
 	PXS_VCOPY(v1, c1); PXS_VCOPY(v2, c2); \
 	_Pragma("unroll") for (int s = 0; s < K; s++) { \
 		const double gp = S.gp2[s], gm = S.gm2[s]; \
-		t0 = fma(gp, tpnr[s], t0); t0 = fma(gm, tpsr[s], t0); \
-		t1 = fma(gp, tpni[s], t1); t1 = fma(gm, tpsi[s], t1); \
-		t2 = fma(gm, tmnr[s], t2); t2 = fma(gp, tmsr[s], t2); \
-		t3 = fma(gm, tmni[s], t3); t3 = fma(gp, tmsi[s], t3); \
+		if (s >= SLO) { \
+			t0 = fma(gp, tpnr[s], t0); t0 = fma(gm, tpsr[s], t0); \
+			t1 = fma(gp, tpni[s], t1); t1 = fma(gm, tpsi[s], t1); \
+			t2 = fma(gm, tmnr[s], t2); t2 = fma(gp, tmsr[s], t2); \
+			t3 = fma(gm, tmni[s], t3); t3 = fma(gp, tmsi[s], t3); \
+		} \
 		S.gp1[s] = fma(fma(ca, S.x[s], v1), gp, -S.gp1[s]); S.gm1[s] = fma(fma(ca, S.x[s], v2), gm, -S.gm1[s]); \
 	} }
 #define SPIN_ANA_STEP1_C(ca, c1, c2) { \
 	PXS_VCOPY(v1, c1); PXS_VCOPY(v2, c2); \
 	_Pragma("unroll") for (int s = 0; s < K; s++) { \
 		const double gp = S.gp1[s], gm = S.gm1[s]; \
-		u0 = fma(gp, tpnr[s], u0); u0 = fma(-gm, tpsr[s], u0); \
-		u1 = fma(gp, tpni[s], u1); u1 = fma(-gm, tpsi[s], u1); \
-		u2 = fma(gm, tmnr[s], u2); u2 = fma(-gp, tmsr[s], u2); \
-		u3 = fma(gm, tmni[s], u3); u3 = fma(-gp, tmsi[s], u3); \
+		if (s >= SLO) { \
+			u0 = fma(gp, tpnr[s], u0); u0 = fma(-gm, tpsr[s], u0); \
+			u1 = fma(gp, tpni[s], u1); u1 = fma(-gm, tpsi[s], u1); \
+			u2 = fma(gm, tmnr[s], u2); u2 = fma(-gp, tmsr[s], u2); \
+			u3 = fma(gm, tmni[s], u3); u3 = fma(-gp, tmsi[s], u3); \
+		} \
 		S.gp2[s] = fma(fma(ca, S.x[s], v1), gp, -S.gp2[s]); S.gm2[s] = fma(fma(ca, S.x[s], v2), gm, -S.gm2[s]); \
 	} }
 #define SPIN_ANA_PAIR_D(ca0, c10, c20, ca1, c11, c21, jfirst, NEXT) { \
@@ -280,19 +292,66 @@
 	LEG_RED_PUT(kk, t0, t1, t2, t3) \
 	LEG_RED_PUT(kk+1, u0, u1, u2, u3) \
 	kk += 2; }
-#define SPIN_ANA_PHASE_C { \
-	spin_rows_t n = spin_rows(coef, j), f = spin_rows(coef, j+1); \
-	PXS_ROWS_DRAIN(); \
-	n.r1 = n.r0; \
-	while (j + 3 < nl) {       \
-		SPIN_ANA_PAIR_R(SPIN_ROW1(n), SPIN_ROW0(f), j, n = spin_rows(coef, j+3)) \
-		SPIN_ANA_PAIR_R(SPIN_ROW1(f), SPIN_ROW0(n), j+2, f = spin_rows(coef, j+5)) \
-		j += 4; \
-	} \
-	if (j + 1 < nl) { \
-		SPIN_ANA_PAIR_R(SPIN_ROW1(n), SPIN_ROW0(f), j, (void)0) \
-		j += 2; \
-	} }
+#define SPIN_ANA_STAGE(NB) if constexpr ((NB) <= K) { if (nb == (NB)) { \
+	constexpr int SLO = K - (NB); \
+	bool more = false; \
+	if (!inC) { \
+	while (j + 1 < nl) { \
+		if constexpr ((NB) < K) if (j < nl && SPIN_BLOCK_STARTS(SLO - 1)) { more = true; break; } \
+		bool pend = false; \
+		_Pragma("unroll") for (int s = 0; s < K; s++) pend |= (S.scp[s] < 0) || (S.scm[s] < 0); \
+		if (!__any(pend)) break; \
+		for (int it = 0; it < 2 && j + 1 < nl; it++, j += 2) { \
+			const double4_t f0 = LDC(coef, j), f1 = LDC(coef, j+1); \
+			SPIN_ANA_PAIR(f0, f1) \
+		} \
+		_Pragma("unroll") for (int s = 0; s < K; s++) { \
+			const bool was = (S.scp[s] < 0) || (S.scm[s] < 0); \
+			if (S.scp[s] < 0 && fabs(S.gp2[s]) > SC_BIG) { S.gp1[s] *= SC_SMALL; S.gp2[s] *= SC_SMALL; S.scp[s]++; } \
+			if (S.scm[s] < 0 && fabs(S.gm2[s]) > SC_BIG) { S.gm1[s] *= SC_SMALL; S.gm2[s] *= SC_SMALL; S.scm[s]++; } \
+			if (s >= SLO && was && S.scp[s] == 0 && S.scm[s] == 0) load_data(s); \
+		} \
+	} \
+	if (!more) { \
+		n = spin_rows(coef, j); f = spin_rows(coef, j+1); \
+		PXS_ROWS_DRAIN(); \
+		n.r1 = n.r0; \
+		inC = 1; \
+	} } \
+	if (!more) { \
+		for (;;) {       \
+			if constexpr ((NB) < K) if (j < nl && SPIN_BLOCK_STARTS(SLO - 1)) { more = true; break; } \
+			if (!(j + 3 < nl)) break; \
+			SPIN_ANA_PAIR_R(SPIN_ROW1(n), SPIN_ROW0(f), j, n = spin_rows(coef, j+3)) \
+			SPIN_ANA_PAIR_R(SPIN_ROW1(f), SPIN_ROW0(n), j+2, f = spin_rows(coef, j+5)) \
+			j += 4; \
+		} \
+	} \
+	if (!more) { \
+		slo = SLO; \
+		nb = K + 1; \
+	} else if constexpr ((NB) < K) { SPIN_BLOCK_BEGIN(SLO - 1) if (S.scp[SLO - 1] == 0 && S.scm[SLO - 1] == 0) load_data(SLO - 1); if constexpr ((NB) + 1 < K) { SPIN_NEXT_START(SLO - 2) } nb = (NB) + 1; } \
+} }
+#define SPIN_ANA_TAIL { const int SLO = slo; \
+		if (j + 1 < nl) { \
+			SPIN_ANA_PAIR_R(SPIN_ROW1(n), SPIN_ROW0(f), j, (void)0) \
+			j += 2; \
+		} \
+		PXS_ROWS_DRAIN(); \
+		if (kk == LEG_FSTEPS) { leg_flush(red, pout + 4*jbase, lane, LEG_FSTEPS, a.atomic); kk = 0; jbase = j; } \
+		if (j < nl) { \
+			double t0 = 0, t1 = 0, t2 = 0, t3 = 0; \
+			_Pragma("unroll") for (int s = 0; s < K; s++) if (s >= SLO) { \
+				const double gp = S.gp2[s], gm = S.gm2[s]; \
+				t0 = fma(gp, tpnr[s], t0); t0 = fma(gm, tpsr[s], t0); \
+				t1 = fma(gp, tpni[s], t1); t1 = fma(gm, tpsi[s], t1); \
+				t2 = fma(gm, tmnr[s], t2); t2 = fma(gp, tmsr[s], t2); \
+				t3 = fma(gm, tmni[s], t3); t3 = fma(gp, tmsi[s], t3); \
+			} \
+			LEG_RED_PUT(kk, t0, t1, t2, t3) \
+			kk++; \
+		} }
+
 #define SPIN_ANA_PAIR_R(s0, s1, jfirst, NEXT) SPIN_ANA_PAIR_D(s0, s1, jfirst, NEXT)
 
 template<int K> __global__ __launch_bounds__(64, (K == 2 ? 5 : 1)) void leg_ana_spin(const LegK a)
@@ -328,44 +387,18 @@
 	int j = 0;
 	SPIN_SEEDED_PHASE_A
 	j = PXS_UNIFORM_INT(j); coef = (const double4_t*)PXS_UNIFORM_LONG((long)coef);
-	PXS_COUNT(1, (long)(nl - j)*K*12 + (a.seed_mode != 2 ? (long)j*K*4 : 0L));
+	constexpr int DIR = 1;
+	PXS_COUNT2(DIR, (long)(nl - j)*K*4 + (a.seed_mode != 2 ? (long)j*K*4 : 0L), (long)(nl - j)*8, K);
+	int knext = LEG_NEVER;
+	if constexpr (K > 1) { SPIN_NEXT_START(K - 2) }
 	if (lane == 0 && !a.atomic) a.first[wv*a.nmc + (m - a.m0)] = j + 1;
-#pragma unroll
-	for (int s = 0; s < K; s++) if (S.scp[s] == 0 && S.scm[s] == 0) load_data(s);
+	if (S.scp[K - 1] == 0 && S.scm[K - 1] == 0) load_data(K - 1);
 	int kk = 0, jbase = j;
-	while (j + 1 < nl) {
-		bool pend = false;
-#pragma unroll
-		for (int s = 0; s < K; s++) pend |= (S.scp[s] < 0) || (S.scm[s] < 0);
-		if (!__any(pend)) break;
-		for (int it = 0; it < 2 && j + 1 < nl; it++, j += 2) {
-			const double4_t f0 = LDC(coef, j), f1 = LDC(coef, j+1);
-			SPIN_ANA_PAIR(f0, f1)
-		}
-#pragma unroll
-		for (int s = 0; s < K; s++) {
-			const bool was = (S.scp[s] < 0) || (S.scm[s] < 0);
-			if (S.scp[s] < 0 && fabs(S.gp2[s]) > SC_BIG) { S.gp1[s] *= SC_SMALL; S.gp2[s] *= SC_SMALL; S.scp[s]++; }
-			if (S.scm[s] < 0 && fabs(S.gm2[s]) > SC_BIG) { S.gm1[s] *= SC_SMALL; S.gm2[s] *= SC_SMALL; S.scm[s]++; }
-			if (was && S.scp[s] == 0 && S.scm[s] == 0) load_data(s);
-		}
-	}
-	SPIN_ANA_PHASE_C
-	PXS_ROWS_DRAIN();
-	if (kk == LEG_FSTEPS) { leg_flush(red, pout + 4*jbase, lane, LEG_FSTEPS, a.atomic); kk = 0; jbase = j; }
-	if (j < nl) {
-		double t0 = 0, t1 = 0, t2 = 0, t3 = 0;
-#pragma unroll
-		for (int s = 0; s < K; s++) {
-			const double gp = S.gp2[s], gm = S.gm2[s];
-			t0 = fma(gp, tpnr[s], t0); t0 = fma(gm, tpsr[s], t0);
-			t1 = fma(gp, tpni[s], t1); t1 = fma(gm, tpsi[s], t1);
-			t2 = fma(gm, tmnr[s], t2); t2 = fma(gp, tmsr[s], t2);
-			t3 = fma(gm, tmni[s], t3); t3 = fma(gp, tmsi[s], t3);
-		}
-		LEG_RED_PUT(kk, t0, t1, t2, t3)
-		kk++;
-	}
+	spin_rows_t n, f;
+	int nb = 1, inC = 0, slo = 0;
+	SPIN_ANA_STAGE(1) SPIN_ANA_STAGE(2) SPIN_ANA_STAGE(3) SPIN_ANA_STAGE(4) SPIN_ANA_STAGE(5) SPIN_ANA_STAGE(6)
+	static_assert(K <= 6, "leg_ana_spin: one SPIN_ANA_STAGE per block");
+	SPIN_ANA_TAIL
 	if (kk > 0) leg_flush(red, pout + 4*jbase, lane, kk, a.atomic);
 }
 
diff --git a/pixell_amd/csrc/legendre_dev.hpp b/pixell_amd/csrc/legendre_dev.hpp
--- a/pixell_amd/csrc/legendre_dev.hpp
+++ b/pixell_amd/csrc/legendre_dev.hpp
@@ -11,6 +11,14 @@
 static constexpr int    SC_STEP  = 800;
 static constexpr double LEG_LIVE = 0x1p-140;
 #define LEG_IS_LIVE(v, sc) ((sc) == 0 && fabs(v) >= LEG_LIVE)
+
+#define LEG_NEVER 0x7fffffff
+template<int C, int K> __device__ __forceinline__ bool leg_live_upto(const double (&v)[K], const int (&sc)[K]) {
+	bool act = false;
+#pragma unroll
+	for (int s = 0; s <= C; s++) act |= LEG_IS_LIVE(v[s], sc[s]);
+	return act;
+}
 
 struct double4_t { double a, b, c, d; };
 #ifdef PXS_HOST_SIM
@@ -75,10 +83,13 @@
 };
 #define PXS_NCOUNT 1024
 #ifdef PXS_HOST_SIM
-#define PXS_COUNT(dir, expr) if (a.count != nullptr && lane == 0) atomicAdd(a.count + 2*(blockIdx.x & (PXS_NCOUNT - 1)) + (dir), (double)(expr))
-#else
-#define PXS_COUNT(dir, expr) if (a.count != nullptr && lane == 0) unsafeAtomicAdd(a.count + 2*(blockIdx.x & (PXS_NCOUNT - 1)) + (dir), (double)(expr))
-#endif
+#define PXS_COUNT_AT(i, expr) if (a.count != nullptr && lane == 0) atomicAdd(a.count + 4*(blockIdx.x & (PXS_NCOUNT - 1)) + (i), (double)(expr))
+#else
+#define PXS_COUNT_AT(i, expr) if (a.count != nullptr && lane == 0) unsafeAtomicAdd(a.count + 4*(blockIdx.x & (PXS_NCOUNT - 1)) + (i), (double)(expr))
+#endif
+#define PXS_COUNT(dir, expr) PXS_COUNT_AT(dir, expr)
+#define PXS_COUNT2(dir, rec, acc, K_) { PXS_COUNT_AT(dir, (rec) + (K_)*(acc)); if ((K_) > 1) PXS_COUNT_AT(2 + (dir), ((K_) - 1)*(acc)); }
+#define PXS_COUNT_BLOCK(dir, acc) PXS_COUNT_AT(2 + (dir), -(acc))
 
 __host__ __device__ constexpr unsigned leg_blocks_per_m(unsigned nwave, unsigned nb) { return (nwave*nb) | 1u; }
 static_assert(leg_blocks_per_m(20, 1) == 21 && leg_blocks_per_m(27, 1) == 27 && leg_blocks_per_m(4, 8) == 33 && leg_blocks_per_m(3, 2) == 7, "blocks per m: odd, at most one more than chunks x maps");
diff --git a/pixell_amd/csrc/sht.hip b/pixell_amd/csrc/sht.hip
--- a/pixell_amd/csrc/sht.hip
+++ b/pixell_amd/csrc/sht.hip
@@ -331,6 +331,15 @@
 	PXS_REQUIRE(p, "pxs_plan_query: null argument");
 	if (p->pts) *value = points_query(p->pts, n);
 	else if (n == "analysis_form") { const Route r = analysis_route_now(p); *value = (r.kind == R_RING_WEIGHTS || r.kind == R_CC_WEIGHTS) ? 1 : (r.form->fine ? 2 : 0); }
+	else if (n == "leg_executed_flops_ana") {
+		double sum = 0;
+		if (p->wk.count.p) {
+			PXS_HIP(hipSetDevice(p->device)); PXS_HIP(hipDeviceSynchronize());
+			std::vector<double> c(p->wk.count.bytes/sizeof(double)); PXS_HIP(hipMemcpy(c.data(), p->wk.count.p, p->wk.count.bytes, hipMemcpyDeviceToHost));
+			for (size_t i = 1; i + 2 < c.size(); i += 4) sum += (c[i] - c[i + 2])*128.0;
+		}
+		*value = (int64_t)sum;
+	}
 	else if (n == "leg_ana_k") *value = p->wk.last_ana_k;
 	else if (n == "ncc_circle") *value = p->th.ncc > 0 ? p->th.Ncc : 0;
 	else if (n == "ducc_ncc_circle") *value = FftChain::ducc_ncc(p->lmax);
@@ -402,7 +411,7 @@
 	PXS_TRY
 	PXS_REQUIRE(p, "pxs_profile: null plan");
 	p->prof.enabled = enable != 0;
-	if (enable && !p->wk.count.p) { PXS_HIP(hipSetDevice(p->device)); p->wk.count.alloc(2*1024*sizeof(double)); PXS_HIP(hipMemset(p->wk.count.p, 0, p->wk.count.bytes)); }
+	if (enable && !p->wk.count.p) { PXS_HIP(hipSetDevice(p->device)); p->wk.count.alloc(4*1024*sizeof(double));  PXS_HIP(hipMemset(p->wk.count.p, 0, p->wk.count.bytes)); }
 	p->wk.count_on = enable != 0;
 	PXS_CATCH
 }
@@ -415,7 +424,7 @@
 	PXS_HIP(hipSetDevice(p->device));
 	PXS_HIP(hipDeviceSynchronize());
 	std::vector<double> c(p->wk.count.bytes/sizeof(double)); PXS_HIP(hipMemcpy(c.data(), p->wk.count.p, p->wk.count.bytes, hipMemcpyDeviceToHost));
-	for (size_t i = 0; i + 1 < c.size(); i += 2) { flops[0] += c[i]*128.0; flops[1] += c[i+1]*128.0; }
+	for (size_t i = 0; i + 3 < c.size(); i += 4) { flops[0] += c[i]*128.0; flops[1] += c[i+1]*128.0; }
 	if (reset) PXS_HIP(hipMemset(p->wk.count.p, 0, p->wk.count.bytes));
 	PXS_CATCH
 }
diff --git a/pixell_amd/sht.py b/pixell_amd/sht.py
--- a/pixell_amd/sht.py
+++ b/pixell_amd/sht.py
@@ -69,10 +69,11 @@
 		_lib.check(_lib.load().pxs_profile_read(self.handle, ms, cnt, int(bool(reset))))
 		names = ["leg_syn", "leg_ana", "ring_fft", "resample"]
 		return {n: (ms[i], cnt[i]) for i, n in enumerate(names)}
-	def profile_flops(self, reset=True):
+	def profile_flops(self, reset=True, executed=False):
+		ana = float(self.query("leg_executed_flops_ana")) if executed else None
 		f = (ctypes.c_double*2)()
 		_lib.check(_lib.load().pxs_profile_flops(self.handle, f, int(bool(reset))))
-		return f[0], f[1]
+		return (f[0], ana) if executed else (f[0], f[1])
 	def set_option(self, name, value):
 		_lib.check(_lib.load().pxs_plan_option(self.handle, name.encode(), int(value)))
 	def query(self, name):
```
